# prannaykaul/lvc

Hardware: AMD Instinct MI355X
Metric: img/s COCO 800x1333 R50-FPN inference (GeneralizedRCNN.forward(batched_inputs) -> Instances, 1000 proposals, 100 detections) (higher is better)
Workload: dtype f32 (conv/GEMM inner products on the fp16 / bf16 matrix cores through fp32-accurate operand splits: two-way fp16 with main + cross fp32 accumulators for the 3x3 and wide 1x1 / FC layers, three-way bf16 for the rest; final boxes/scores closer to the fp64 evaluation than the reference's fp32 CPU path,; 1 GPU; COCO-detection R50-FPN inference, bs=8 synthetic 3x800x1333 per GPU, 1000 pre/post-NMS proposals per level/image, 80 classes, conditioned random-init weights; batch_per_gpu=8, global_batch=8, parallelism=dp1

## Files before the change

lvc_amd/_lib.py:

```python
import ctypes
import os

_HERE = os.path.dirname(os.path.abspath(__file__))
_SO = os.environ.get("LVC_AMD_LIB") or os.path.join(_HERE, "liblvc_amd.so")
_lib = None

c_void_p = ctypes.c_void_p
c_int = ctypes.c_int
c_float = ctypes.c_float
c_double = ctypes.c_double
c_longlong = ctypes.c_longlong


class LvcNativeError(RuntimeError):
    pass


def lib():
    global _lib
    if _lib is None:
        if not os.path.exists(_SO):
            raise ImportError(
                "lvc_amd: native library {} not found; build it with "
                "`python -c 'import __graft_entry__ as g; g.build()'` or `make -C lvc_amd/csrc` "
                "(there is no CPU fallback)".format(_SO)
            )
        L = ctypes.CDLL(_SO)
        L.lvc_last_error.restype = ctypes.c_char_p
        L.lvc_batched_nms_workspace_bytes.restype = c_longlong
        L.lvc_tta_merge_workspace_bytes.restype = c_longlong
        L.lvc_abi_version.restype = c_int
        L.lvc_set_wino_streamk.restype = None
        if os.environ.get("LVC_WINO_STREAMK", "0") != "0":
            L.lvc_set_wino_streamk(c_int(int(os.environ["LVC_WINO_STREAMK"])))
        L.lvc_set_nms_reduce_global.restype = None
        L.lvc_set_halo_test_hooks.restype = None
        if os.environ.get("LVC_NMS_REDUCE_GLOBAL", "0") != "0":
            L.lvc_set_nms_reduce_global(c_int(1))
        _lib = L
    return _lib


def check(status, what=""):
    if status != 0:
        msg = lib().lvc_last_error().decode("utf-8", "replace")
        lib().lvc_set_range_slot(0)
        raise LvcNativeError("{} failed (status {}): {}".format(what or "lvc_amd native call", status, msg))


def ptr(t):
    if t is None:
        return c_void_p(0)
    return c_void_p(t.data_ptr())


def current_stream(device=None):
    import torch

    return c_void_p(torch.cuda.current_stream(device).cuda_stream)
```

lvc_amd/csrc/boxes.hip:

```cpp
#include "common.h"
#include <stdlib.h>

typedef unsigned long long u64;

extern "C" int lvc_batched_nms(const float*, const float*, const int*, const int*, int, int, double, int,
                               int*, int*, void*, long long, void*);
extern "C" long long lvc_batched_nms_workspace_bytes(int, int);

#define MAXL 8

__device__ __forceinline__ unsigned int desc_key(float f) {
  if (f == 0.f) f = 0.f;
  unsigned int u = __float_as_uint(f);
  u ^= (u >> 31) ? 0xFFFFFFFFu : 0x80000000u;
  return ~u;
}

__device__ __forceinline__ int block_excl_scan_1024(int v, int* sh, int* total) {
  const int lane = threadIdx.x & 63, wave = threadIdx.x >> 6;
  int x = v;
#pragma unroll
  for (int o = 1; o < 64; o <<= 1) {
    int t = __shfl_up(x, o);
    if (lane >= o) x += t;
  }
  __syncthreads();
  if (lane == 63) sh[wave] = x;
  __syncthreads();
  if (threadIdx.x == 0) {
    int s = 0;
    for (int w = 0; w < 16; ++w) { int t = sh[w]; sh[w] = s; s += t; }
    sh[16] = s;
  }
  __syncthreads();
  *total = sh[16];
  return sh[wave] + x - v;
}

template <typename T>
__device__ __forceinline__ void bitonic_sort_lds(T* keys, int npad) {
  for (int k = 2; k <= npad; k <<= 1) {
    for (int j = k >> 1; j > 0; j >>= 1) {
      for (int t = threadIdx.x; t < npad / 2; t += blockDim.x) {
        int lo = ((t & ~(j - 1)) << 1) | (t & (j - 1));
        int hi = lo | j;
        bool up = (lo & k) == 0;
        T a = keys[lo], b = keys[hi];
        if ((a > b) == up) { keys[lo] = b; keys[hi] = a; }
      }
      __syncthreads();
    }
  }
}

struct RpnLevels {
  const float* logits[MAXL];
  const float* deltas[MAXL];
  int ld_logit[MAXL], ld_delta[MAXL];
  int H[MAXL], W[MAXL], stride[MAXL];
  int cand_off[MAXL + 1];
  long long key_off[MAXL + 1];
  const float* cell_anchors[MAXL];
  int L, A;
};

__device__ __forceinline__ void find_digit(const int* __restrict__ h, int krem, int* sh) {
  const int tid = threadIdx.x, lane = tid & 63, wave = tid >> 6;
  int x = 0, incl = 0;
  if (tid < 256) {
    x = h[tid];
    incl = x;
#pragma unroll
    for (int o = 1; o < 64; o <<= 1) {
      const int t = __shfl_up(incl, o);
      if (lane >= o) incl += t;
    }
    if (lane == 63) sh[wave] = incl;
  }
  __syncthreads();
  if (tid < 256) {
    int off = 0;
    for (int w = 0; w < wave; ++w) off += sh[w];
    incl += off;
    if (incl - x < krem && krem <= incl) { sh[8] = tid; sh[9] = incl - x; }
  }
  __syncthreads();
}

#define TOPK_PAD 2048
__global__ __launch_bounds__(1024) void rpn_topk_kernel(RpnLevels lv, int topk, unsigned int* __restrict__ wkeys,
                                                        float* __restrict__ cand_score,
                                                        int* __restrict__ cand_idx, int Ntot, int small_only) {
  __shared__ u64 sortbuf[TOPK_PAD];
  __shared__ int hist[256];
  __shared__ int sh[20];
  __shared__ int s_nlt;
  const int l = blockIdx.x, b = blockIdx.y, tid = threadIdx.x;
  const int A = lv.A, HW = lv.H[l] * lv.W[l], n = HW * A;
  if (n > small_only) return;
  const int k = topk < n ? topk : n;
  const int ld = lv.ld_logit[l];
  const float* lg = lv.logits[l] + (size_t)b * HW * ld;
  unsigned int* keys = wkeys + (size_t)b * lv.key_off[lv.L] + lv.key_off[l];
  const int npad = k <= 1024 ? 1024 : TOPK_PAD;

  if (tid < 256) hist[tid] = 0;
  __syncthreads();
  for (int i = tid; i < n; i += 1024) {
    int p = i / A, a = i - p * A;
    unsigned int key = desc_key(lg[(size_t)p * ld + a]);
    keys[i] = key;
    atomicAdd(&hist[key >> 24], 1);
  }
  __syncthreads();
  unsigned int prefix = 0, pmask = 0;
  int krem = k;
  for (int pass = 0; pass < 4; ++pass) {
    const int shift = 24 - 8 * pass;
    if (pass > 0) {
      if (tid < 256) hist[tid] = 0;
      __syncthreads();
      for (int i = tid; i < n; i += 1024) {
        unsigned int key = keys[i];
        if ((key & pmask) == prefix) atomicAdd(&hist[(key >> shift) & 255], 1);
      }
      __syncthreads();
    }
    find_digit(hist, krem, sh);
    prefix |= (unsigned int)sh[8] << shift;
    pmask |= 255u << shift;
    krem -= sh[9];
    __syncthreads();
  }
  const unsigned int T = prefix;
  const int need_eq = krem, n_lt = k - krem;
  for (int i = tid; i < npad; i += 1024) sortbuf[i] = ~0ull;
  if (tid == 0) s_nlt = 0;
  __syncthreads();
  int eq_base = 0;
  for (int i0 = 0; i0 < n; i0 += 1024) {
    const int i = i0 + tid;
    unsigned int key = i < n ? keys[i] : 0xFFFFFFFFu;
    bool is_lt = i < n && key < T;
    bool is_eq = i < n && key == T;
    if (is_lt) {
      int slot = atomicAdd(&s_nlt, 1);
      sortbuf[slot] = ((u64)key << 32) | (unsigned)i;
    }
    if (eq_base < need_eq) {
      int tot;
      int rank = eq_base + block_excl_scan_1024(is_eq ? 1 : 0, sh, &tot);
      if (is_eq && rank < need_eq) sortbuf[n_lt + rank] = ((u64)key << 32) | (unsigned)i;
      eq_base += tot;
    }
  }
  __syncthreads();
  bitonic_sort_lds(sortbuf, npad);
  for (int r = tid; r < k; r += 1024) {
    int i = (int)(sortbuf[r] & 0xFFFFFFFFu);
    int p = i / A, a = i - p * A;
    cand_idx[(size_t)b * Ntot + lv.cand_off[l] + r] = i;
    cand_score[(size_t)b * Ntot + lv.cand_off[l] + r] = lg[(size_t)p * ld + a];
  }
}

#define TK_SLICE 8192
#define TK_HSTRIDE 1040

__device__ __forceinline__ void topk_prefix(const int* __restrict__ H, int npass, int k, int* sh, unsigned int* prefix,
                                            int* krem) {
  unsigned int pf = 0;
  int kr = k;
  for (int ps = 0; ps < npass; ++ps) {
    find_digit(H + ps * 256, kr, sh);
    pf |= (unsigned int)sh[8] << (24 - 8 * ps);
    kr -= sh[9];
    __syncthreads();
  }
  *prefix = pf;
  *krem = kr;
}

__global__ __launch_bounds__(1024) void rpn_topk_phase_kernel(RpnLevels lv, int topk, unsigned int* __restrict__ wkeys,
                                                              int* __restrict__ hist_all, u64* __restrict__ ckeys,
                                                              int* __restrict__ ties, int Ntot, int phase) {
  __shared__ int hist[256];
  __shared__ int sh[16];
  const int slice = blockIdx.x, l = blockIdx.y, b = blockIdx.z, tid = threadIdx.x, lane = tid & 63;
  const int A = lv.A, HW = lv.H[l] * lv.W[l], n = HW * A;
  if (n <= TK_SLICE) return;
  const int i0 = slice * TK_SLICE;
  if (i0 >= n) return;
  const int i1 = min(n, i0 + TK_SLICE);
  const int k = topk < n ? topk : n;
  const int ld = lv.ld_logit[l];
  const float* lg = lv.logits[l] + (size_t)b * HW * ld;
  unsigned int* keys = wkeys + (size_t)b * lv.key_off[lv.L] + lv.key_off[l];
  int* H = hist_all + ((size_t)b * lv.L + l) * TK_HSTRIDE;
  unsigned int prefix;
  int krem;
  topk_prefix(H, phase < 4 ? phase : 4, k, sh, &prefix, &krem);
  if (phase < 4) {
    if (tid < 256) hist[tid] = 0;
    __syncthreads();
    const unsigned int pmask = phase ? 0xFFFFFFFFu << (32 - 8 * phase) : 0u;
    const int shift = 24 - 8 * phase;
    for (int ib = i0; ib < i1; ib += 1024) {
      const int i = ib + tid;
      unsigned int key = 0;
      bool act = false;
      if (i < i1) {
        if (phase == 0) {
          const int pp = i / A, a = i - pp * A;
          key = desc_key(lg[(size_t)pp * ld + a]);
          keys[i] = key;
        } else {
          key = keys[i];
        }
        act = (key & pmask) == prefix;
      }
      const unsigned int d = (key >> shift) & 255u;
      u64 m = __ballot(act);
      while (m) {
        const int first = __ffsll((long long)m) - 1;
        const unsigned int dd = (unsigned int)__shfl((int)d, first);
        const u64 same = __ballot(act && d == dd);
        if (lane == first) atomicAdd(&hist[dd], __popcll(same));
        m &= ~same;
      }
    }
    __syncthreads();
    if (tid < 256 && hist[tid]) atomicAdd(&H[phase * 256 + tid], hist[tid]);
  } else {
    const unsigned int T = prefix;
    u64* ck = ckeys + (size_t)b * Ntot + lv.cand_off[l];
    int* tl = ties + ((size_t)b * lv.L + l) * TOPK_PAD;
    for (int i = i0 + tid; i < i1; i += 1024) {
      const unsigned int key = keys[i];
      if (key < T) {
        const int slot = atomicAdd(&H[1024], 1);
        ck[slot] = ((u64)key << 32) | (unsigned)i;
      } else if (key == T) {
        const int slot = atomicAdd(&H[1025], 1);
        if (slot < TOPK_PAD) tl[slot] = i;
      }
    }
  }
}

__global__ __launch_bounds__(1024) void rpn_topk_final_kernel(RpnLevels lv, int topk, const unsigned int* __restrict__ wkeys,
                                                              const int* __restrict__ hist_all,
                                                              const u64* __restrict__ ckeys, const int* __restrict__ ties,
                                                              float* __restrict__ cand_score, int* __restrict__ cand_idx,
                                                              int Ntot) {
  __shared__ u64 sortbuf[TOPK_PAD];
  __shared__ unsigned int tiebuf[TOPK_PAD];
  __shared__ int sh[20];
  const int l = blockIdx.x, b = blockIdx.y, tid = threadIdx.x;
  const int A = lv.A, HW = lv.H[l] * lv.W[l], n = HW * A;
  if (n <= TK_SLICE) return;
  const int k = topk < n ? topk : n;
  const int ld = lv.ld_logit[l];
  const float* lg = lv.logits[l] + (size_t)b * HW * ld;
  const unsigned int* keys = wkeys + (size_t)b * lv.key_off[lv.L] + lv.key_off[l];
  const int* H = hist_all + ((size_t)b * lv.L + l) * TK_HSTRIDE;
  unsigned int T;
  int need_eq;
  topk_prefix(H, 4, k, sh, &T, &need_eq);
  const int n_lt = k - need_eq;
  const int npad = k <= 1024 ? 1024 : TOPK_PAD;
  const u64* ck = ckeys + (size_t)b * Ntot + lv.cand_off[l];
  for (int i = tid; i < npad; i += 1024) sortbuf[i] = i < n_lt ? ck[i] : ~0ull;
  const int tie_total = H[1025];
  __syncthreads();
  if (tie_total <= TOPK_PAD) {
    const int* tl = ties + ((size_t)b * lv.L + l) * TOPK_PAD;
    int tp = 64;
    while (tp < tie_total) tp <<= 1;
    for (int i = tid; i < tp; i += 1024) tiebuf[i] = i < tie_total ? (unsigned int)tl[i] : 0xFFFFFFFFu;
    __syncthreads();
    bitonic_sort_lds(tiebuf, tp);
    for (int r = tid; r < need_eq; r += 1024) sortbuf[n_lt + r] = ((u64)T << 32) | tiebuf[r];
  } else {
    int eq_base = 0;
    for (int i0 = 0; i0 < n && eq_base < need_eq; i0 += 1024) {
      const int i = i0 + tid;
      const bool is_eq = i < n && keys[i] == T;
      int tot;
      const int rank = eq_base + block_excl_scan_1024(is_eq ? 1 : 0, sh, &tot);
      if (is_eq && rank < need_eq) sortbuf[n_lt + rank] = ((u64)T << 32) | (unsigned)i;
      eq_base += tot;
    }
  }
  __syncthreads();
  bitonic_sort_lds(sortbuf, npad);
  for (int r = tid; r < k; r += 1024) {
    const int i = (int)(sortbuf[r] & 0xFFFFFFFFu);
    const int pp = i / A, a = i - pp * A;
    cand_idx[(size_t)b * Ntot + lv.cand_off[l] + r] = i;
    cand_score[(size_t)b * Ntot + lv.cand_off[l] + r] = lg[(size_t)pp * ld + a];
  }
}

__device__ __forceinline__ void apply_deltas(float bx1, float by1, float bx2, float by2, float d0, float d1,
                                             float d2, float d3, float wx, float wy, float ww, float wh,
                                             float scale_clamp, float* o) {
  const float widths = bx2 - bx1, heights = by2 - by1;
  const float ctr_x = bx1 + 0.5f * widths, ctr_y = by1 + 0.5f * heights;
  const float dx = d0 / wx, dy = d1 / wy;
  float dw = d2 / ww, dh = d3 / wh;
  dw = dw > scale_clamp ? scale_clamp : dw;
  dh = dh > scale_clamp ? scale_clamp : dh;
  const float pcx = dx * widths + ctr_x, pcy = dy * heights + ctr_y;
  const float pw = expf(dw) * widths, ph = expf(dh) * heights;
  o[0] = pcx - 0.5f * pw; o[1] = pcy - 0.5f * ph; o[2] = pcx + 0.5f * pw; o[3] = pcy + 0.5f * ph;
}
__device__ __forceinline__ float clampf(float v, float lo, float hi) {
  v = v < lo ? lo : v;
  return v > hi ? hi : v;
}


__global__ __launch_bounds__(1024) void rpn_decode_seg_kernel(RpnLevels lv, const float* __restrict__ cand_score,
                                                              const int* __restrict__ cand_idx, int Ntot,
                                                              const int* __restrict__ image_sizes, float scale_clamp,
                                                              float min_box_size, int SN, float* __restrict__ sboxes,
                                                              float* __restrict__ sscores, int* __restrict__ scount) {
  __shared__ int sh[20];
  const int l = blockIdx.x, b = blockIdx.y, tid = threadIdx.x;
  const int seg = b * lv.L + l;
  const float img_h = (float)image_sizes[b * 2 + 0], img_w = (float)image_sizes[b * 2 + 1];
  const int c_begin = lv.cand_off[l], c_end = lv.cand_off[l + 1];
  const int A = lv.A, W = lv.W[l], HW = lv.H[l] * W;
  int base = 0;
  for (int c0 = c_begin; c0 < c_end; c0 += 1024) {
    const int c = c0 + tid;
    bool ok = false;
    float box[4] = {0, 0, 0, 0};
    float score = 0.f;
    if (c < c_end) {
      const int i = cand_idx[(size_t)b * Ntot + c];
      score = cand_score[(size_t)b * Ntot + c];
      const int p = i / A, a = i - p * A;
      const int y = p / W, x = p - y * W;
      const float sx = (float)(x * lv.stride[l]), sy = (float)(y * lv.stride[l]);
      const float* ca = lv.cell_anchors[l] + a * 4;
      const float ax1 = sx + ca[0], ay1 = sy + ca[1], ax2 = sx + ca[2], ay2 = sy + ca[3];
      const float* d = lv.deltas[l] + ((size_t)b * HW + p) * lv.ld_delta[l] + a * 4;
      apply_deltas(ax1, ay1, ax2, ay2, d[0], d[1], d[2], d[3], 1.f, 1.f, 1.f, 1.f, scale_clamp, box);
      ok = isfinite(box[0]) && isfinite(box[1]) && isfinite(box[2]) && isfinite(box[3]) && isfinite(score);
      box[0] = clampf(box[0], 0.f, img_w); box[1] = clampf(box[1], 0.f, img_h);
      box[2] = clampf(box[2], 0.f, img_w); box[3] = clampf(box[3], 0.f, img_h);
      ok = ok && (box[2] - box[0] > min_box_size) && (box[3] - box[1] > min_box_size);
    }
    int tot;
    const int pos = base + block_excl_scan_1024(ok ? 1 : 0, sh, &tot);
    if (ok) {
      float* o = sboxes + ((size_t)seg * SN + pos) * 4;
      o[0] = box[0]; o[1] = box[1]; o[2] = box[2]; o[3] = box[3];
      sscores[(size_t)seg * SN + pos] = score;
    }
    base += tot;
  }
  if (tid == 0) scount[seg] = base;
}

#define MERGE_LDS_SCORES 8192
__global__ __launch_bounds__(1024) void rpn_merge_levels_kernel(const float* __restrict__ sboxes,
                                                                const float* __restrict__ sscores,
                                                                const int* __restrict__ keep,
                                                                const int* __restrict__ num_keep, int L, int SN,
                                                                int post_topk, float* __restrict__ pboxes,
                                                                float* __restrict__ plogits, int* __restrict__ out_count) {
  __shared__ int s_nk[MAXL + 1];
  __shared__ float s_sc[MERGE_LDS_SCORES];
  const int b = blockIdx.x, tid = threadIdx.x;
  if (tid == 0) {
    int acc = 0;
    for (int l = 0; l < L; ++l) { s_nk[l] = acc; acc += num_keep[b * L + l]; }
    s_nk[L] = acc;
  }
  __syncthreads();
  const int total = s_nk[L];
  const int nout = total < post_topk ? total : post_topk;
  const bool in_lds = total <= MERGE_LDS_SCORES;
  if (in_lds) {
    for (int e = tid; e < total; e += 1024) {
      int l = 0;
      while (e >= s_nk[l + 1]) ++l;
      const int seg = b * L + l;
      s_sc[e] = sscores[(size_t)seg * SN + keep[(size_t)seg * SN + (e - s_nk[l])]];
    }
    __syncthreads();
  }
  for (int e = tid; e < total; e += 1024) {
    int l = 0;
    while (e >= s_nk[l + 1]) ++l;
    const int t = e - s_nk[l];
    const int seg = b * L + l;
    const int j = keep[(size_t)seg * SN + t];
    const float s = sscores[(size_t)seg * SN + j];
    int rank = t;
    for (int m = 0; m < L; ++m) {
      if (m == l) continue;
      const int segm = b * L + m, n = s_nk[m + 1] - s_nk[m];
      int lo = 0, hi = n;
      while (lo < hi) {
        const int mid = (lo + hi) >> 1;
        const float sm = in_lds ? s_sc[s_nk[m] + mid] : sscores[(size_t)segm * SN + keep[(size_t)segm * SN + mid]];
        if (sm > s || (sm == s && m < l)) lo = mid + 1; else hi = mid;
      }
      rank += lo;
    }
    if (rank < post_topk) {
      *reinterpret_cast<float4*>(pboxes + ((size_t)b * post_topk + rank) * 4) =
          *reinterpret_cast<const float4*>(sboxes + ((size_t)seg * SN + j) * 4);
      plogits[(size_t)b * post_topk + rank] = s;
    }
  }
  for (int r = nout + tid; r < post_topk; r += 1024) {
    *reinterpret_cast<float4*>(pboxes + ((size_t)b * post_topk + r) * 4) = float4{0.f, 0.f, 0.f, 0.f};
    plogits[(size_t)b * post_topk + r] = 0.f;
  }
  if (tid == 0) out_count[b] = nout;
}


static long long align16(long long x) { return (x + 15) & ~15ll; }

struct RpnPlan {
  int Ntot;
  long long nkeys;
  long long off_keys, off_cscore, off_cidx, off_cboxes, off_cscores2, off_clevels, off_ccount, off_keep, off_hist, off_ckeys, off_ties, off_nms, total;
  long long off_sboxes, off_sscores, off_scount, off_skeep, off_snk, off_snms, snms_bytes;
  int max_slices, SN;
};
static RpnPlan rpn_plan(int B, int L, int A, const int* Hs, const int* Ws, int pre_topk) {
  RpnPlan p;
  p.Ntot = 0; p.nkeys = 0; p.max_slices = 0;
  for (int l = 0; l < L; ++l) {
    long long n = (long long)Hs[l] * Ws[l] * A;
    p.nkeys += n;
    p.Ntot += (int)(n < pre_topk ? n : pre_topk);
    if (n > TK_SLICE) { int sl = (int)((n + TK_SLICE - 1) / TK_SLICE); if (sl > p.max_slices) p.max_slices = sl; }
  }
  long long o = 0;
  p.off_keys = o; o = align16(o + (long long)B * p.nkeys * 4);
  p.off_cscore = o; o = align16(o + (long long)B * p.Ntot * 4);
  p.off_cidx = o; o = align16(o + (long long)B * p.Ntot * 4);
  p.off_cboxes = o; o = align16(o + (long long)B * p.Ntot * 16);
  p.off_cscores2 = o; o = align16(o + (long long)B * p.Ntot * 4);
  p.off_clevels = o; o = align16(o + (long long)B * p.Ntot * 4);
  p.off_ccount = o; o = align16(o + (long long)B * 4);
  p.off_keep = o; o = align16(o + (long long)B * p.Ntot * 4);
  p.off_hist = o; o = align16(o + (long long)B * L * TK_HSTRIDE * 4);
  p.off_ckeys = o; o = align16(o + (long long)B * p.Ntot * 8);
  p.off_ties = o; o = align16(o + (long long)B * L * TOPK_PAD * 4);
  p.off_nms = o; o = align16(o + lvc_batched_nms_workspace_bytes(B, p.Ntot));
  p.SN = 0;
  for (int l = 0; l < L; ++l) {
    long long n = (long long)Hs[l] * Ws[l] * A;
    const int c = (int)(n < pre_topk ? n : pre_topk);
    if (c > p.SN) p.SN = c;
  }
  const long long segs = (long long)B * L;
  p.off_sboxes = o; o = align16(o + segs * p.SN * 16);
  p.off_sscores = o; o = align16(o + segs * p.SN * 4);
  p.off_scount = o; o = align16(o + segs * 4);
  p.off_skeep = o; o = align16(o + segs * p.SN * 4);
  p.off_snk = o; o = align16(o + segs * 4);
  p.snms_bytes = lvc_batched_nms_workspace_bytes((int)segs, p.SN);
  p.off_snms = o; o = align16(o + p.snms_bytes);
  p.total = o;
  return p;
}

extern "C" long long lvc_rpn_proposals_workspace_bytes(int B, int L, int A, const int* Hs, const int* Ws,
                                                       int pre_nms_topk) {
  if (L < 1 || L > MAXL) return -1;
  return rpn_plan(B, L, A, Hs, Ws, pre_nms_topk).total;
}

extern "C" int lvc_rpn_proposals(const float* const* logits, const int* ld_logit, const float* const* deltas,
                                 const int* ld_delta, const float* const* cell_anchors, const int* Hs,
                                 const int* Ws, const int* strides, int L, int A, int B,
                                 const int* d_image_sizes, int pre_nms_topk, int post_nms_topk,
                                 double nms_thresh, float min_box_size, float scale_clamp,
                                 float* out_boxes, float* out_logits, int* d_out_count, void* workspace,
                                 long long workspace_bytes, void* stream) {
  LVC_CHECK_ARG(L >= 1 && L <= MAXL, "1..8 levels");
  LVC_CHECK_ARG(B > 0 && A > 0, "bad B/A");
  LVC_CHECK_ARG(pre_nms_topk > 0 && pre_nms_topk <= TOPK_PAD, "pre_nms_topk must be in 1..2048");
  LVC_CHECK_ARG(post_nms_topk > 0, "post_nms_topk must be positive");
  LVC_CHECK_ARG(logits && deltas && cell_anchors && Hs && Ws && strides && d_image_sizes && out_boxes &&
                    out_logits && d_out_count && workspace, "null pointer");
  RpnPlan p = rpn_plan(B, L, A, Hs, Ws, pre_nms_topk);
  LVC_CHECK_ARG(workspace_bytes >= p.total, "workspace too small");
  RpnLevels lv;
  memset(&lv, 0, sizeof lv);
  lv.L = L; lv.A = A;
  for (int l = 0; l < L; ++l) {
    lv.logits[l] = logits[l]; lv.deltas[l] = deltas[l];
    lv.ld_logit[l] = ld_logit[l]; lv.ld_delta[l] = ld_delta[l];
    lv.H[l] = Hs[l]; lv.W[l] = Ws[l]; lv.stride[l] = strides[l];
    lv.cell_anchors[l] = cell_anchors[l];
    long long n = (long long)Hs[l] * Ws[l] * A;
    lv.key_off[l + 1] = lv.key_off[l] + n;
    lv.cand_off[l + 1] = lv.cand_off[l] + (int)(n < pre_nms_topk ? n : pre_nms_topk);
  }
  char* ws = (char*)workspace;
  hipStream_t st = (hipStream_t)stream;
  unsigned int* keys = (unsigned int*)(ws + p.off_keys);
  float* cand_score = (float*)(ws + p.off_cscore);
  int* cand_idx = (int*)(ws + p.off_cidx);
  const bool multi = p.max_slices > 0;
  if (multi) {
    int* hist = (int*)(ws + p.off_hist);
    u64* ckeys = (u64*)(ws + p.off_ckeys);
    int* ties = (int*)(ws + p.off_ties);
    if (hipMemsetAsync(hist, 0, (size_t)B * L * TK_HSTRIDE * 4, st) != hipSuccess) {
      lvc_set_error("%s: hipMemsetAsync failed", __func__);
      return LVC_ERR_HIP;
    }
    for (int phase = 0; phase <= 4; ++phase)
      hipLaunchKernelGGL(rpn_topk_phase_kernel, dim3(p.max_slices, L, B), dim3(1024), 0, st, lv, pre_nms_topk, keys,
                         hist, ckeys, ties, p.Ntot, phase);
    hipLaunchKernelGGL(rpn_topk_final_kernel, dim3(L, B), dim3(1024), 0, st, lv, pre_nms_topk, keys, hist, ckeys, ties,
                       cand_score, cand_idx, p.Ntot);
  }
  hipLaunchKernelGGL(rpn_topk_kernel, dim3(L, B), dim3(1024), 0, st, lv, pre_nms_topk, keys, cand_score,
                     cand_idx, p.Ntot, multi ? TK_SLICE : 0x7FFFFFFF);
  LVC_CHECK_LAUNCH();
  float* sboxes = (float*)(ws + p.off_sboxes);
  float* sscores = (float*)(ws + p.off_sscores);
  int* scount = (int*)(ws + p.off_scount);
  int* skeep = (int*)(ws + p.off_skeep);
  int* snk = (int*)(ws + p.off_snk);
  hipLaunchKernelGGL(rpn_decode_seg_kernel, dim3(L, B), dim3(1024), 0, st, lv, cand_score, cand_idx, p.Ntot,
                     d_image_sizes, scale_clamp, min_box_size, p.SN, sboxes, sscores, scount);
  LVC_CHECK_LAUNCH();
  const int keep_per_level = post_nms_topk < p.SN ? post_nms_topk : p.SN;
  int rc = lvc_batched_nms(sboxes, sscores, nullptr, scount, B * L, p.SN, nms_thresh, keep_per_level, skeep, snk,
                           ws + p.off_snms, p.snms_bytes, stream);
  if (rc) return rc;
  hipLaunchKernelGGL(rpn_merge_levels_kernel, dim3(B), dim3(1024), 0, st, sboxes, sscores, skeep, snk, L, p.SN,
                     post_nms_topk, out_boxes, out_logits, d_out_count);
  LVC_CHECK_LAUNCH();
  return LVC_OK;
}

__global__ void assign_levels_kernel(const float* __restrict__ boxes, int R, int B, int min_level, int max_level,
                                     float canonical_box_size, float canonical_level, int* __restrict__ levels,
                                     float* __restrict__ rois) {
  const int i = blockIdx.x * blockDim.x + threadIdx.x;
  if (i >= R * B) return;
  const float4 bx = *reinterpret_cast<const float4*>(boxes + (size_t)i * 4);
  const float area = (bx.z - bx.x) * (bx.w - bx.y);
  const float size = sqrtf(area);
  float lvl = floorf(canonical_level + log2f(size / canonical_box_size + 1e-8f));
  lvl = lvl < (float)min_level ? (float)min_level : lvl;
  lvl = lvl > (float)max_level ? (float)max_level : lvl;
  levels[i] = (int)lvl - min_level;
  if (rois) {
    float* r = rois + (size_t)i * 5;
    r[0] = (float)(i / R); r[1] = bx.x; r[2] = bx.y; r[3] = bx.z; r[4] = bx.w;
  }
}

extern "C" int lvc_assign_levels_rois(const float* boxes, int B, int R, int min_level, int max_level,
                                      int canonical_box_size, int canonical_level, int* levels, float* rois,
                                      void* stream) {
  LVC_CHECK_ARG(B >= 0 && R >= 0, "negative size");
  if (B * R == 0) return LVC_OK;
  LVC_CHECK_ARG(boxes && levels, "null pointer");
  hipLaunchKernelGGL(assign_levels_kernel, dim3(lvc_cdiv(B * R, 256)), dim3(256), 0, (hipStream_t)stream, boxes, R,
                     B, min_level, max_level, (float)canonical_box_size, (float)canonical_level, levels, rois);
  LVC_CHECK_LAUNCH();
  return LVC_OK;
}

#define DET_TILE_ROWS 64
#define DET_MAX_COLS 97
__global__ __launch_bounds__(DET_TILE_ROWS) void det_row_stats_kernel(const float* __restrict__ cls_logits, int ld_cls, int K,
                                                                     int rows, float score_thresh, float* __restrict__ st_mx,
                                                                     float* __restrict__ st_inv, int* __restrict__ st_cnt,
                                                                     unsigned long long* __restrict__ st_mask) {
  __shared__ float tile[DET_TILE_ROWS * DET_MAX_COLS];
  const int r0 = blockIdx.x * DET_TILE_ROWS, tid = threadIdx.x;
  const int ncol = K + 1, pitch = ncol | 1;
  for (int i = tid; i < DET_TILE_ROWS * ncol; i += DET_TILE_ROWS) {
    const int rr = i / ncol, cc = i - rr * ncol;
    const int r = r0 + rr;
    tile[rr * pitch + cc] = r < rows ? cls_logits[(size_t)r * ld_cls + cc] : 0.f;
  }
  __syncthreads();
  const int r = r0 + tid;
  if (r >= rows) return;
  const float* lg = tile + tid * pitch;
  float mx = -INFINITY;
  for (int k = 0; k <= K; ++k) { float v = lg[k]; mx = v > mx ? v : mx; }
  float sum = 0.f;
  for (int k = 0; k <= K; ++k) sum += expf(lg[k] - mx);
  const float inv = 1.f / sum;
  int cnt = 0;
  unsigned long long m0 = 0, m1 = 0;
  for (int k = 0; k < K; ++k) {
    const bool hit = expf(lg[k] - mx) * inv > score_thresh;
    cnt += hit ? 1 : 0;
    if (hit) { if (k < 64) m0 |= 1ull << k; else m1 |= 1ull << (k - 64); }
  }
  st_mx[r] = mx; st_inv[r] = inv; st_cnt[r] = cnt;
  st_mask[2 * (size_t)r] = m0; st_mask[2 * (size_t)r + 1] = m1;
}

__global__ __launch_bounds__(1024) void det_candidates_kernel(
    const float* __restrict__ cls_logits, int ld_cls, const float* __restrict__ deltas, int ld_delta,
    int K, int cls_agnostic, const float* __restrict__ proposals, const int* __restrict__ prop_count, int R,
    const int* __restrict__ image_sizes, float wx, float wy, float ww, float wh, float scale_clamp,
    float score_thresh, int Nmax, float* __restrict__ cboxes, float* __restrict__ cscores,
    int* __restrict__ cclass, int* __restrict__ crow, int* __restrict__ ccount, int* __restrict__ status,
    const float* __restrict__ st_mx, const float* __restrict__ st_inv, const int* __restrict__ st_cnt,
    const unsigned long long* __restrict__ st_mask) {
  __shared__ int sh[20];
  const int b = blockIdx.x, tid = threadIdx.x;
  const int nrow = prop_count ? min(prop_count[b], R) : R;
  const float img_h = (float)image_sizes[b * 2 + 0], img_w = (float)image_sizes[b * 2 + 1];
  int base = 0;
  for (int r0 = 0; r0 < nrow; r0 += 1024) {
    const int r = r0 + tid;
    int cnt = 0;
    float mx = -INFINITY, inv = 0.f;
    const float* lg = cls_logits + ((size_t)b * R + (r < nrow ? r : 0)) * ld_cls;
    if (r < nrow && st_cnt) {
      const size_t gr = (size_t)b * R + r;
      mx = st_mx[gr]; inv = st_inv[gr]; cnt = st_cnt[gr];
    } else if (r < nrow) {
      for (int k = 0; k <= K; ++k) { float v = lg[k]; mx = v > mx ? v : mx; }
      float sum = 0.f;
      for (int k = 0; k <= K; ++k) sum += expf(lg[k] - mx);
      inv = 1.f / sum;
      for (int k = 0; k < K; ++k) cnt += (expf(lg[k] - mx) * inv > score_thresh) ? 1 : 0;
    }
    int tot;
    int pos = base + block_excl_scan_1024(cnt, sh, &tot);
    if (r < nrow && cnt > 0) {
      const float4 pb = *reinterpret_cast<const float4*>(proposals + ((size_t)b * R + r) * 4);
      const float* dl = deltas + ((size_t)b * R + r) * ld_delta;
      auto emit = [&](int k) {
        const float pr = expf(lg[k] - mx) * inv;
        if (pr > score_thresh) {
          if (pos < Nmax) {
            const float* d = dl + (cls_agnostic ? 0 : k * 4);
            float box[4];
            apply_deltas(pb.x, pb.y, pb.z, pb.w, d[0], d[1], d[2], d[3], wx, wy, ww, wh, scale_clamp, box);
            float* o = cboxes + ((size_t)b * Nmax + pos) * 4;
            o[0] = clampf(box[0], 0.f, img_w); o[1] = clampf(box[1], 0.f, img_h);
            o[2] = clampf(box[2], 0.f, img_w); o[3] = clampf(box[3], 0.f, img_h);
            cscores[(size_t)b * Nmax + pos] = pr;
            cclass[(size_t)b * Nmax + pos] = k;
            crow[(size_t)b * Nmax + pos] = r;
          }
          ++pos;
        }
      };
      if (st_mask) {
        for (int w = 0; w < 2; ++w) {
          unsigned long long m = st_mask[2 * ((size_t)b * R + r) + w];
          while (m) {
            emit(w * 64 + __ffsll((long long)m) - 1);
            m &= m - 1;
          }
        }
      } else {
        for (int k = 0; k < K; ++k) emit(k);
      }
    }
    base += tot;
  }
  if (tid == 0) {
    if (base > Nmax) { atomicOr(status, 2); base = Nmax; }
    ccount[b] = base;
  }
}

__global__ __launch_bounds__(256) void det_gather_kernel(
    const float* __restrict__ cboxes, const float* __restrict__ cscores, const int* __restrict__ cclass,
    const int* __restrict__ crow, const int* __restrict__ keep, const int* __restrict__ num_keep, int Nmax,
    int topk, const float* __restrict__ post, float* __restrict__ oboxes, float* __restrict__ oscores,
    int* __restrict__ oclasses, int* __restrict__ orows, int* __restrict__ ocount) {
  __shared__ int wsum[4];
  const int b = blockIdx.x, tid = threadIdx.x;
  const int nk = min(num_keep[b], topk);
  int base = 0;
  for (int r0 = 0; r0 < topk; r0 += 256) {
    const int r = r0 + tid;
    bool ok = false;
    float4 bx = {0, 0, 0, 0};
    float s = 0.f; int c = 0, row = 0;
    if (r < nk) {
      const int i = keep[(size_t)b * Nmax + r];
      bx = *reinterpret_cast<const float4*>(cboxes + ((size_t)b * Nmax + i) * 4);
      s = cscores[(size_t)b * Nmax + i]; c = cclass[(size_t)b * Nmax + i]; row = crow[(size_t)b * Nmax + i];
      ok = true;
      if (post) {
        const float sx = post[b * 4 + 0], sy = post[b * 4 + 1], oh = post[b * 4 + 2], ow = post[b * 4 + 3];
        bx.x = clampf(bx.x * sx, 0.f, ow); bx.y = clampf(bx.y * sy, 0.f, oh);
        bx.z = clampf(bx.z * sx, 0.f, ow); bx.w = clampf(bx.w * sy, 0.f, oh);
        ok = (bx.z - bx.x > 0.f) && (bx.w - bx.y > 0.f);
      }
    }
    const u64 bal = __ballot(ok);
    const int lane = tid & 63, wave = tid >> 6;
    __syncthreads();
    if (lane == 0) wsum[wave] = __popcll(bal);
    __syncthreads();
    int wbase = 0, tot = 0;
    for (int w = 0; w < 4; ++w) { if (w < wave) wbase += wsum[w]; tot += wsum[w]; }
    const int pos = base + wbase + __popcll(bal & ((1ull << lane) - 1ull));
    if (ok) {
      *reinterpret_cast<float4*>(oboxes + ((size_t)b * topk + pos) * 4) = bx;
      oscores[(size_t)b * topk + pos] = s; oclasses[(size_t)b * topk + pos] = c; orows[(size_t)b * topk + pos] = row;
    }
    base += tot;
  }
  __syncthreads();
  for (int r = base + tid; r < topk; r += 256) {
    float4 z = {0, 0, 0, 0};
    *reinterpret_cast<float4*>(oboxes + ((size_t)b * topk + r) * 4) = z;
    oscores[(size_t)b * topk + r] = 0.f; oclasses[(size_t)b * topk + r] = 0; orows[(size_t)b * topk + r] = 0;
  }
  if (tid == 0) ocount[b] = base;
}

struct DetPlan { long long off_cboxes, off_cscores, off_cclass, off_crow, off_ccount, off_keep, off_nk, off_nms, total; };
static DetPlan det_plan(int B, int Nmax) {
  DetPlan p; long long o = 0;
  p.off_cboxes = o; o = align16(o + (long long)B * Nmax * 16);
  p.off_cscores = o; o = align16(o + (long long)B * Nmax * 4);
  p.off_cclass = o; o = align16(o + (long long)B * Nmax * 4);
  p.off_crow = o; o = align16(o + (long long)B * Nmax * 4);
  p.off_ccount = o; o = align16(o + (long long)B * 4);
  p.off_keep = o; o = align16(o + (long long)B * Nmax * 4);
  p.off_nk = o; o = align16(o + (long long)B * 4);
  p.off_nms = o; o = align16(o + lvc_batched_nms_workspace_bytes(B, Nmax));
  p.total = o;
  return p;
}
extern "C" long long lvc_fast_rcnn_inference_workspace_bytes(int B, int max_candidates) {
  return det_plan(B, max_candidates).total;
}

extern "C" int lvc_fast_rcnn_inference(const float* cls_logits, int ld_cls, const float* deltas, int ld_delta,
                                       int K, int cls_agnostic, const float* proposals,
                                       const int* d_prop_count, int B, int R, const int* d_image_sizes,
                                       float wx, float wy, float ww, float wh, float scale_clamp,
                                       float score_thresh, double nms_thresh, int topk, int max_candidates,
                                       const float* d_post, float* out_boxes, float* out_scores,
                                       int* out_classes, int* out_rows, int* d_out_count, int* d_status,
                                       void* workspace, long long workspace_bytes, void* stream) {
  LVC_CHECK_ARG(B > 0 && R > 0 && K > 0 && topk > 0, "bad sizes");
  LVC_CHECK_ARG(max_candidates > 0, "max_candidates must be positive");
  LVC_CHECK_ARG(cls_logits && deltas && proposals && d_image_sizes && out_boxes && out_scores && out_classes &&
                    out_rows && d_out_count && d_status && workspace, "null pointer");
  DetPlan p = det_plan(B, max_candidates);
  LVC_CHECK_ARG(workspace_bytes >= p.total, "workspace too small");
  char* ws = (char*)workspace;
  hipStream_t st = (hipStream_t)stream;
  float* cboxes = (float*)(ws + p.off_cboxes);
  float* cscores = (float*)(ws + p.off_cscores);
  int* cclass = (int*)(ws + p.off_cclass);
  int* crow = (int*)(ws + p.off_crow);
  int* ccount = (int*)(ws + p.off_ccount);
  int* keep = (int*)(ws + p.off_keep);
  int* nk = (int*)(ws + p.off_nk);
  const long long rows = (long long)B * R;
  float* st_mx = nullptr; float* st_inv = nullptr; int* st_cnt = nullptr;
  unsigned long long* st_mask = nullptr;
  if (K + 1 < DET_MAX_COLS && rows * 28 + 64 <= p.total - p.off_nms) {
    st_mask = (unsigned long long*)(ws + p.off_nms);
    st_mx = (float*)(st_mask + 2 * rows);
    st_inv = st_mx + rows;
    st_cnt = (int*)(st_inv + rows);
    hipLaunchKernelGGL(det_row_stats_kernel, dim3((unsigned)lvc_cdiv64(rows, DET_TILE_ROWS)), dim3(DET_TILE_ROWS), 0, st,
                       cls_logits, ld_cls, K, (int)rows, score_thresh, st_mx, st_inv, st_cnt, st_mask);
    LVC_CHECK_LAUNCH();
  }
  hipLaunchKernelGGL(det_candidates_kernel, dim3(B), dim3(1024), 0, st, cls_logits, ld_cls, deltas, ld_delta, K,
                     cls_agnostic, proposals, d_prop_count, R, d_image_sizes, wx, wy, ww, wh, scale_clamp,
                     score_thresh, max_candidates, cboxes, cscores, cclass, crow, ccount, d_status, st_mx, st_inv, st_cnt, st_mask);
  LVC_CHECK_LAUNCH();
  int rc = lvc_batched_nms(cboxes, cscores, cclass, ccount, B, max_candidates, nms_thresh, topk, keep, nk,
                           ws + p.off_nms, p.total - p.off_nms, stream);
  if (rc) return rc;
  hipLaunchKernelGGL(det_gather_kernel, dim3(B), dim3(256), 0, st, cboxes, cscores, cclass, crow, keep, nk,
                     max_candidates, topk, d_post, out_boxes, out_scores, out_classes, out_rows, d_out_count);
  LVC_CHECK_LAUNCH();
  return LVC_OK;
}

__global__ void decode_boxes_kernel(const float* __restrict__ deltas, int ld, const float* __restrict__ boxes, int M,
                                    int R, const int* __restrict__ image_sizes, float wx, float wy, float ww, float wh,
                                    float scale_clamp, float* __restrict__ out) {
  const int i = blockIdx.x * blockDim.x + threadIdx.x;
  if (i >= M) return;
  const float4 b = *reinterpret_cast<const float4*>(boxes + (size_t)i * 4);
  const float* d = deltas + (size_t)i * ld;
  float o[4];
  apply_deltas(b.x, b.y, b.z, b.w, d[0], d[1], d[2], d[3], wx, wy, ww, wh, scale_clamp, o);
  if (image_sizes) {
    const int img = i / R;
    const float h = (float)image_sizes[img * 2], w = (float)image_sizes[img * 2 + 1];
    o[0] = clampf(o[0], 0.f, w); o[1] = clampf(o[1], 0.f, h); o[2] = clampf(o[2], 0.f, w); o[3] = clampf(o[3], 0.f, h);
  }
  float4 r = {o[0], o[1], o[2], o[3]};
  *reinterpret_cast<float4*>(out + (size_t)i * 4) = r;
}

extern "C" int lvc_decode_boxes(const float* deltas, int ld, const float* boxes, int M, int R, const int* d_image_sizes,
                                float wx, float wy, float ww, float wh, float scale_clamp, float* out, void* stream) {
  LVC_CHECK_ARG(M >= 0 && R > 0 && ld >= 4, "bad shape");
  if (M == 0) return LVC_OK;
  LVC_CHECK_ARG(deltas && boxes && out, "null pointer");
  hipLaunchKernelGGL(decode_boxes_kernel, dim3(lvc_cdiv(M, 256)), dim3(256), 0, (hipStream_t)stream, deltas, ld, boxes, M, R,
                     d_image_sizes, wx, wy, ww, wh, scale_clamp, out);
  LVC_CHECK_LAUNCH();
  return LVC_OK;
}
```

lvc_amd/csrc/nms.hip:

```cpp
#include "common.h"

typedef unsigned long long u64;

__device__ __forceinline__ unsigned int ordered_desc_key(float f) {
  if (f == 0.f) f = 0.f;
  unsigned int u = __float_as_uint(f);
  u ^= (u >> 31) ? 0xFFFFFFFFu : 0x80000000u;
  return ~u;
}

template <int NPAD>
__global__ __launch_bounds__(1024) void nms_prep_kernel(const float* __restrict__ boxes,
                                                        const float* __restrict__ scores,
                                                        const int* __restrict__ idxs,
                                                        const int* __restrict__ counts, int Nmax,
                                                        int* __restrict__ order,
                                                        float* __restrict__ sboxes,
                                                        int* __restrict__ sidx) {
  extern __shared__ __attribute__((aligned(16))) unsigned char dsm[];
  u64* keys = reinterpret_cast<u64*>(dsm);
  __shared__ float red[16];
  const int img = blockIdx.x;
  const int tid = threadIdx.x;
  int n = counts ? counts[img] : Nmax;
  if (n > Nmax) n = Nmax;
  const float* bx = boxes + (size_t)img * Nmax * 4;
  const float* sc = scores + (size_t)img * Nmax;
  const int* ix = idxs ? idxs + (size_t)img * Nmax : nullptr;

  float m = -INFINITY;
  for (int i = tid; i < n * 4; i += 1024) {
    float v = bx[i];
    m = v > m ? v : m;
  }
  for (int o = 32; o > 0; o >>= 1) {
    float t = __shfl_xor(m, o);
    m = t > m ? t : m;
  }
  if ((tid & 63) == 0) red[tid >> 6] = m;
  __syncthreads();
  if (tid < 64) {
    float v = tid < 16 ? red[tid] : -INFINITY;
    for (int o = 8; o > 0; o >>= 1) {
      float t = __shfl_xor(v, o);
      v = t > v ? t : v;
    }
    if (tid == 0) red[0] = v;
  }
  __syncthreads();
  const float maxp1 = red[0] + 1.0f;

  int npad = 1024;
  while (npad < n) npad <<= 1;
  if (npad > NPAD) npad = NPAD;
  for (int i = tid; i < npad; i += 1024)
    keys[i] = i < n ? (((u64)ordered_desc_key(sc[i]) << 32) | (unsigned)i) : ~0ull;
  __syncthreads();
  for (int k = 2; k <= npad; k <<= 1) {
    for (int j = k >> 1; j > 0; j >>= 1) {
      for (int t = tid; t < npad / 2; t += 1024) {
        int lo = ((t & ~(j - 1)) << 1) | (t & (j - 1));
        int hi = lo | j;
        bool up = (lo & k) == 0;
        u64 a = keys[lo], b = keys[hi];
        if ((a > b) == up) { keys[lo] = b; keys[hi] = a; }
      }
      __syncthreads();
    }
  }
  int* ord = order + (size_t)img * Nmax;
  float* sb = sboxes + (size_t)img * Nmax * 4;
  int* si = sidx + (size_t)img * Nmax;
  for (int r = tid; r < n; r += 1024) {
    int i = (int)(keys[r] & 0xFFFFFFFFu);
    ord[r] = i;
    int id = ix ? ix[i] : 0;
    float off = (float)id * maxp1;
    sb[r * 4 + 0] = bx[i * 4 + 0] + off;
    sb[r * 4 + 1] = bx[i * 4 + 1] + off;
    sb[r * 4 + 2] = bx[i * 4 + 2] + off;
    sb[r * 4 + 3] = bx[i * 4 + 3] + off;
    si[r] = id;
  }
}

#define NMS_MASK_STRIDE 96
#define NMS_TILE 16384
#define NMS_HEAD_MIN 2048
__global__ __launch_bounds__(64) void nms_mask_kernel(const float* __restrict__ sboxes,
                                                      const int* __restrict__ sidx,
                                                      const int* __restrict__ counts, int Nmax,
                                                      int nwords, double thr, u64* __restrict__ mask, int row0,
                                                      int rows_cap, const int* __restrict__ num_keep, int max_keep) {
  const int img = blockIdx.z;
  int n = counts ? counts[img] : Nmax;
  if (n > Nmax) n = Nmax;
  const int nend = n < row0 + rows_cap ? n : row0 + rows_cap;
  if (num_keep && num_keep[img] >= max_keep) return;
  const int nchunks = nend > row0 ? (nend - row0 + 63) >> 6 : 0;
  const int lane = threadIdx.x;
  const float* sb = sboxes + (size_t)img * Nmax * 4;
  const int* si = sidx + (size_t)img * Nmax;
  for (int ci = blockIdx.y; ci < nchunks; ci += gridDim.y) {
  const int i_me = row0 + ci * 64 + lane;
  float ix1 = 0, iy1 = 0, ix2 = 0, iy2 = 0; int iid = -1;
  if (i_me < nend) {
    const float4 b = *reinterpret_cast<const float4*>(sb + (size_t)i_me * 4);
    ix1 = b.x; iy1 = b.y; ix2 = b.z; iy2 = b.w; iid = si[i_me];
  }
  const float iarea_me = (ix2 - ix1) * (iy2 - iy1);
  const int rows = min(64, nend - (row0 + ci * 64));
  for (int wj = ci + blockIdx.x; wj < nchunks; wj += gridDim.x) {
    const int j_me = row0 + wj * 64 + lane;
    float jx1 = 0, jy1 = 0, jx2 = 0, jy2 = 0; int jid = -2;
    if (j_me < nend) {
      const float4 b = *reinterpret_cast<const float4*>(sb + (size_t)j_me * 4);
      jx1 = b.x; jy1 = b.y; jx2 = b.z; jy2 = b.w; jid = si[j_me];
    }
    const float jarea = (jx2 - jx1) * (jy2 - jy1);
    u64 my_word = 0;
    for (int r = 0; r < rows; ++r) {
      const float ax1 = __shfl(ix1, r), ay1 = __shfl(iy1, r), ax2 = __shfl(ix2, r), ay2 = __shfl(iy2, r);
      const float aarea = __shfl(iarea_me, r);
      const int aid = __shfl(iid, r);
      const float xx1 = ax1 < jx1 ? jx1 : ax1;
      const float yy1 = ay1 < jy1 ? jy1 : ay1;
      const float xx2 = jx2 < ax2 ? jx2 : ax2;
      const float yy2 = jy2 < ay2 ? jy2 : ay2;
      float w = xx2 - xx1; if (!(w > 0.f)) w = 0.f;
      float h = yy2 - yy1; if (!(h > 0.f)) h = 0.f;
      const float inter = w * h;
      const float ovr = inter / (aarea + jarea - inter);
      const bool hit = (j_me < nend) && (j_me != row0 + ci * 64 + r) && (aid == jid) && ((double)ovr > thr);
      const u64 word = __ballot(hit);
      if (lane == r) my_word = word;
    }
    if (i_me < nend) mask[((size_t)img * rows_cap + (i_me - row0)) * nwords + wj] = my_word;
  }
  }
}

__global__ __launch_bounds__(256) void nms_cross_kernel(const float* __restrict__ sboxes, const int* __restrict__ sidx,
                                                        const int* __restrict__ counts, int Nmax, int nwords, double thr,
                                                        const int* __restrict__ kept_pos, const int* __restrict__ num_keep,
                                                        int max_keep, int row0, int rows_cap, u64* __restrict__ removed_init) {
  const int w = blockIdx.x * 4 + (threadIdx.x >> 6), lane = threadIdx.x & 63, img = blockIdx.y;
  if (w >= nwords) return;
  int n = counts ? counts[img] : Nmax;
  if (n > Nmax) n = Nmax;
  const int nend = n < row0 + rows_cap ? n : row0 + rows_cap;
  const int nk = num_keep[img];
  u64* dst = removed_init + (size_t)img * nwords + w;
  if (row0 + w * 64 >= nend || nk >= max_keep) {
    if (lane == 0) *dst = 0ull;
    return;
  }
  const float* sb = sboxes + (size_t)img * Nmax * 4;
  const int* si = sidx + (size_t)img * Nmax;
  const int* kp = kept_pos + (size_t)img * Nmax;
  const int j_me = row0 + w * 64 + lane;
  float jx1 = 0, jy1 = 0, jx2 = 0, jy2 = 0; int jid = -2;
  if (j_me < nend) {
    const float4 b = *reinterpret_cast<const float4*>(sb + (size_t)j_me * 4);
    jx1 = b.x; jy1 = b.y; jx2 = b.z; jy2 = b.w; jid = si[j_me];
  }
  const float jarea = (jx2 - jx1) * (jy2 - jy1);
  bool dead = false;
  for (int i = 0; i < nk; ++i) {
    const int p = kp[i];
    const float4 a = *reinterpret_cast<const float4*>(sb + (size_t)p * 4);
    const int aid = si[p];
    const float aarea = (a.z - a.x) * (a.w - a.y);
    const float xx1 = a.x < jx1 ? jx1 : a.x;
    const float yy1 = a.y < jy1 ? jy1 : a.y;
    const float xx2 = jx2 < a.z ? jx2 : a.z;
    const float yy2 = jy2 < a.w ? jy2 : a.w;
    float ww = xx2 - xx1; if (!(ww > 0.f)) ww = 0.f;
    float hh = yy2 - yy1; if (!(hh > 0.f)) hh = 0.f;
    const float inter = ww * hh;
    const float ovr = inter / (aarea + jarea - inter);
    dead = dead || ((aid == jid) && ((double)ovr > thr));
  }
  const u64 word = __ballot(dead && j_me < nend);
  if (lane == 0) *dst = word;
}

#define NMS_MAX_WORDS 256
__global__ __launch_bounds__(64) void nms_reduce_kernel(const u64* __restrict__ mask,
                                                        const int* __restrict__ order,
                                                        const int* __restrict__ counts, int Nmax,
                                                        int nwords, int max_keep,
                                                        int* __restrict__ keep,
                                                        int* __restrict__ num_keep, int row0, int rows_cap,
                                                        const u64* __restrict__ removed_init, int* __restrict__ kept_pos,
                                                        int accumulate) {
  __shared__ u64 removed[NMS_MAX_WORDS];
  const int img = blockIdx.x, lane = threadIdx.x;
  int n = counts ? counts[img] : Nmax;
  if (n > Nmax) n = Nmax;
  const int nend = n < row0 + rows_cap ? n : row0 + rows_cap;
  int nk = accumulate ? num_keep[img] : 0;
  if (accumulate && (row0 >= nend || nk >= max_keep)) return;
  const u64* mk = mask + (size_t)img * rows_cap * nwords;
  const int* ord = order + (size_t)img * Nmax;
  int* kp = keep + (size_t)img * Nmax;
  int* kpos = kept_pos ? kept_pos + (size_t)img * Nmax : nullptr;
  for (int w = lane; w < nwords; w += 64) removed[w] = (removed_init && row0 > 0) ? removed_init[(size_t)img * nwords + w] : 0ull;
  __syncthreads();
  const int nchunks = nend > row0 ? (nend - row0 + 63) >> 6 : 0;
  for (int c = 0; c < nchunks && nk < max_keep; ++c) {
    const int row = row0 + c * 64 + lane;
    const u64 diag = row < nend ? mk[(size_t)(row - row0) * nwords + c] : 0ull;
    u64 alive = ~removed[c];
    const int valid = nend - (row0 + c * 64);
    if (valid < 64) alive &= ((1ull << valid) - 1ull);
    alive = ((u64)(unsigned)__builtin_amdgcn_readfirstlane((int)(unsigned)(alive >> 32)) << 32) |
            (unsigned)__builtin_amdgcn_readfirstlane((int)(unsigned)alive);
    const u64 col = diag & ((1ull << lane) - 1ull);
    u64 kept = 0;
    while (alive) {
      const bool und = (alive >> lane) & 1ull;
      const bool rem = und && (col & kept) != 0ull;
      const bool kp1 = und && !rem && (col & alive) == 0ull;
      const u64 bk = __ballot(kp1), br = __ballot(rem);
      kept |= bk;
      alive &= ~(bk | br);
    }
    if ((kept >> lane) & 1ull) {
      const int pos = nk + __popcll(kept & ((1ull << lane) - 1ull));
      if (pos < max_keep) {
        kp[pos] = ord[row];
        if (kpos) kpos[pos] = row;
      }
    }
    nk += __popcll(kept);
    for (int w0 = c + 1; w0 < nchunks; w0 += 64) {
      const int w = w0 + lane;
      const int wc = w < nwords ? w : nwords - 1;
      u64 acc = 0;
      u64 k = kept;
      while (k) {
        u64 v[24];
#pragma unroll
        for (int u = 0; u < 24; ++u) {
          const int i = k ? __ffsll((long long)k) - 1 : -1;
          k &= k - 1;
          const u64 x = mk[(size_t)(c * 64 + (i < 0 ? 0 : i)) * nwords + wc];
          v[u] = i < 0 ? 0ull : x;
        }
#pragma unroll
        for (int u = 0; u < 24; ++u) acc |= v[u];
      }
      if (w < nwords) removed[w] |= acc;
    }
    __syncthreads();
  }
  if (lane == 0) num_keep[img] = nk < max_keep ? nk : max_keep;
}

#define NMS_LDS_ROWS 1024
#define NMS_LDS_PITCH 17
__global__ __launch_bounds__(256) void nms_reduce_lds_kernel(const u64* __restrict__ mask, const int* __restrict__ order,
                                                             const int* __restrict__ counts, int Nmax, int nwords, int max_keep,
                                                             int* __restrict__ keep, int* __restrict__ num_keep, int rows_cap) {
  __shared__ u64 m[NMS_LDS_ROWS * NMS_LDS_PITCH];
  __shared__ int sord[NMS_LDS_ROWS];
  const int img = blockIdx.x, tid = threadIdx.x, lane = tid & 63;
  int n = counts ? counts[img] : Nmax;
  if (n > Nmax) n = Nmax;
  if (n > rows_cap) n = rows_cap;
  const u64* mk = mask + (size_t)img * rows_cap * nwords;
  const int* ord = order + (size_t)img * Nmax;
  const int nchunks = (n + 63) >> 6;
  for (int r = tid; r < n; r += 256) sord[r] = ord[r];
  const int total = n * nwords;
  for (int base = tid; base < total; base += 256 * 8) {
    u64 v[8];
#pragma unroll
    for (int j = 0; j < 8; ++j) {
      const int idx = base + j * 256;
      v[j] = idx < total ? mk[idx] : 0ull;
    }
#pragma unroll
    for (int j = 0; j < 8; ++j) {
      const int idx = base + j * 256;
      const int r = idx / nwords, w = idx - r * nwords;
      if (idx < total && w >= (r >> 6) && w < nchunks) m[r * NMS_LDS_PITCH + w] = v[j];
    }
  }
  __syncthreads();
  if (tid >= 64) return;
  int* kp = keep + (size_t)img * Nmax;
  u64 removed = 0;
  int nk = 0;
  const int w16 = lane & 15, g4 = lane >> 4;
  for (int c = 0; c < nchunks && nk < max_keep; ++c) {
    const int row = c * 64 + lane;
    const u64 diag = row < n ? m[row * NMS_LDS_PITCH + c] : 0ull;
    const u64 rem_c = ((u64)(unsigned)__builtin_amdgcn_readlane((int)(unsigned)(removed >> 32), c) << 32) |
                      (unsigned)__builtin_amdgcn_readlane((int)(unsigned)removed, c);
    u64 alive = ~rem_c;
    const int valid = n - c * 64;
    if (valid < 64) alive &= ((1ull << valid) - 1ull);
    const u64 col = diag & ((1ull << lane) - 1ull);
    u64 kept = 0;
    while (alive) {
      const bool und = (alive >> lane) & 1ull;
      const bool rem = und && (col & kept) != 0ull;
      const bool kp1 = und && !rem && (col & alive) == 0ull;
      const u64 bk = __ballot(kp1), br = __ballot(rem);
      kept |= bk;
      alive &= ~(bk | br);
    }
    if ((kept >> lane) & 1ull) {
      const int pos = nk + __popcll(kept & ((1ull << lane) - 1ull));
      if (pos < max_keep) kp[pos] = sord[row];
    }
    nk += __popcll(kept);
    if (c + 1 < nchunks) {
      u64 acc = 0;
#pragma unroll
      for (int i = 0; i < 64; i += 4) {
        const int r = i + g4;
        const u64 x = m[(c * 64 + r) * NMS_LDS_PITCH + w16];
        acc |= ((kept >> r) & 1ull) ? x : 0ull;
      }
      acc |= (u64)__shfl_xor((long long)acc, 16);
      acc |= (u64)__shfl_xor((long long)acc, 32);
      if (lane < 16 && lane > c) removed |= acc;
    }
  }
  if (lane == 0) num_keep[img] = nk < max_keep ? nk : max_keep;
}

__device__ __forceinline__ unsigned int ordered_asc_key(float f) {
  unsigned int u = __float_as_uint(f);
  return u ^ ((u >> 31) ? 0xFFFFFFFFu : 0x80000000u);
}
__device__ __forceinline__ float ordered_asc_value(unsigned int u) {
  u ^= (u >> 31) ? 0x80000000u : 0xFFFFFFFFu;
  return __uint_as_float(u);
}

__global__ __launch_bounds__(256) void nms_max_kernel(const float* __restrict__ boxes, const int* __restrict__ counts,
                                                      int Nmax, unsigned int* __restrict__ maxkey) {
  const int img = blockIdx.y;
  int n = counts ? counts[img] : Nmax;
  if (n > Nmax) n = Nmax;
  const float* bx = boxes + (size_t)img * Nmax * 4;
  float m = -INFINITY;
  for (int i = blockIdx.x * 256 + threadIdx.x; i < n * 4; i += gridDim.x * 256) {
    const float v = bx[i];
    m = v > m ? v : m;
  }
  for (int o = 32; o > 0; o >>= 1) {
    const float t = __shfl_xor(m, o);
    m = t > m ? t : m;
  }
  if ((threadIdx.x & 63) == 0) atomicMax(maxkey + img, ordered_asc_key(m));
}

__global__ __launch_bounds__(1024) void nms_sort_tile_kernel(const float* __restrict__ scores, const int* __restrict__ counts,
                                                             int Nmax, int npad, u64* __restrict__ keys, int mode, int klevel) {
  extern __shared__ __attribute__((aligned(16))) unsigned char dsm[];
  u64* tk = reinterpret_cast<u64*>(dsm);
  const int img = blockIdx.y, tile = blockIdx.x, tid = threadIdx.x;
  int n = counts ? counts[img] : Nmax;
  if (n > Nmax) n = Nmax;
  if (mode == 1 && n <= (klevel >> 1)) return;
  const int base = tile * NMS_TILE;
  u64* gk = keys + (size_t)img * npad + base;
  if (mode == 0) {
    const float* sc = scores + (size_t)img * Nmax;
    for (int i = tid; i < NMS_TILE; i += 1024) {
      const int gi = base + i;
      tk[i] = gi < n ? (((u64)ordered_desc_key(sc[gi]) << 32) | (unsigned)gi) : ~0ull;
    }
  } else {
    for (int i = tid; i < NMS_TILE; i += 1024) tk[i] = gk[i];
  }
  __syncthreads();
  const int k0 = mode == 0 ? 2 : klevel, k1 = mode == 0 ? NMS_TILE : klevel;
  for (int k = k0; k <= k1; k <<= 1) {
    for (int j = (k >> 1) < NMS_TILE ? (k >> 1) : (NMS_TILE >> 1); j > 0; j >>= 1) {
      for (int t = tid; t < NMS_TILE / 2; t += 1024) {
        const int lo = ((t & ~(j - 1)) << 1) | (t & (j - 1));
        const int hi = lo | j;
        const bool up = ((base + lo) & k) == 0;
        const u64 a = tk[lo], b = tk[hi];
        if ((a > b) == up) { tk[lo] = b; tk[hi] = a; }
      }
      __syncthreads();
    }
  }
  for (int i = tid; i < NMS_TILE; i += 1024) gk[i] = tk[i];
}

__global__ __launch_bounds__(256) void nms_sort_global_kernel(const int* __restrict__ counts, int Nmax, int npad,
                                                              u64* __restrict__ keys, int k, int j) {
  const int img = blockIdx.y;
  int n = counts ? counts[img] : Nmax;
  if (n > Nmax) n = Nmax;
  if (n <= (k >> 1)) return;
  u64* gk = keys + (size_t)img * npad;
  for (int t = blockIdx.x * 256 + threadIdx.x; t < npad / 2; t += gridDim.x * 256) {
    const int lo = ((t & ~(j - 1)) << 1) | (t & (j - 1));
    const int hi = lo | j;
    const bool up = (lo & k) == 0;
    const u64 a = gk[lo], b = gk[hi];
    if ((a > b) == up) { gk[lo] = b; gk[hi] = a; }
  }
}

__global__ __launch_bounds__(256) void nms_gather_kernel(const float* __restrict__ boxes, const int* __restrict__ idxs,
                                                         const int* __restrict__ counts, int Nmax, int npad,
                                                         const u64* __restrict__ keys, const unsigned int* __restrict__ maxkey,
                                                         int* __restrict__ order, float* __restrict__ sboxes,
                                                         int* __restrict__ sidx) {
  const int img = blockIdx.y;
  int n = counts ? counts[img] : Nmax;
  if (n > Nmax) n = Nmax;
  const float maxp1 = ordered_asc_value(maxkey[img]) + 1.0f;
  const float* bx = boxes + (size_t)img * Nmax * 4;
  const int* ix = idxs ? idxs + (size_t)img * Nmax : nullptr;
  const u64* gk = keys + (size_t)img * npad;
  int* ord = order + (size_t)img * Nmax;
  float* sb = sboxes + (size_t)img * Nmax * 4;
  int* si = sidx + (size_t)img * Nmax;
  for (int r = blockIdx.x * 256 + threadIdx.x; r < n; r += gridDim.x * 256) {
    const int i = (int)(gk[r] & 0xFFFFFFFFu);
    ord[r] = i;
    const int id = ix ? ix[i] : 0;
    const float off = (float)id * maxp1;
    sb[(size_t)r * 4 + 0] = bx[(size_t)i * 4 + 0] + off;
    sb[(size_t)r * 4 + 1] = bx[(size_t)i * 4 + 1] + off;
    sb[(size_t)r * 4 + 2] = bx[(size_t)i * 4 + 2] + off;
    sb[(size_t)r * 4 + 3] = bx[(size_t)i * 4 + 3] + off;
    si[r] = id;
  }
}

static int pad_pow2(int n) {
  int p = 1024;
  while (p < n) p <<= 1;
  return p;
}

static long long pad_pow2_ll(long long n) {
  long long p = NMS_TILE;
  while (p < n) p <<= 1;
  return p;
}

extern "C" long long lvc_batched_nms_workspace_bytes(int B, int Nmax) {
  const long long rows = Nmax < NMS_TILE ? Nmax : NMS_TILE;
  const long long nwords = (rows + 63) / 64;
  long long per = (long long)Nmax * 4 * 4  + (long long)Nmax * 4  +
                  (long long)Nmax * 4  + rows * nwords * 8 ;
  if (Nmax > NMS_TILE)
    per += (long long)Nmax * 4 + NMS_MAX_WORDS * 8 + pad_pow2_ll(Nmax) * 8 + 16;
  else if (Nmax > NMS_HEAD_MIN)
    per += (long long)Nmax * 4 + NMS_MAX_WORDS * 8 + 16;
  return (long long)B * per + 512;
}

static int g_nms_reduce_global = 0;
extern "C" void lvc_set_nms_reduce_global(int on) { g_nms_reduce_global = on; }

extern "C" int lvc_batched_nms(const float* boxes, const float* scores, const int* idxs,
                               const int* d_counts, int B, int Nmax, double iou_threshold,
                               int max_keep, int* keep, int* d_num_keep, void* workspace,
                               long long workspace_bytes, void* stream) {
  LVC_CHECK_ARG(B >= 0 && Nmax >= 0, "negative size");
  if (B == 0) return LVC_OK;
  LVC_CHECK_ARG(d_num_keep, "null d_num_keep");
  hipStream_t st = (hipStream_t)stream;
  if (Nmax == 0) {
    (void)hipMemsetAsync(d_num_keep, 0, sizeof(int) * B, st);
    return LVC_OK;
  }
  LVC_CHECK_ARG(boxes && scores && keep && workspace, "null pointer");
  LVC_CHECK_ARG(workspace_bytes >= lvc_batched_nms_workspace_bytes(B, Nmax), "workspace too small");
  LVC_CHECK_ARG(((uintptr_t)workspace & 15) == 0, "workspace must be 16-byte aligned");
  const int rows_cap = Nmax < NMS_TILE ? Nmax : NMS_TILE;
  const int nwords = (rows_cap + 63) / 64;
  char* ws = (char*)workspace;
  float* sboxes = (float*)ws; ws += (size_t)B * Nmax * 16;
  int* order = (int*)ws; ws += (size_t)B * Nmax * 4;
  int* sidx = (int*)ws; ws += (size_t)B * Nmax * 4;
  ws = (char*)(((uintptr_t)ws + 15) & ~(uintptr_t)15);
  u64* mask = (u64*)ws; ws += (size_t)B * rows_cap * nwords * 8;
  if (max_keep <= 0) max_keep = Nmax;
  const dim3 mask_grid(nwords < NMS_MASK_STRIDE ? nwords : NMS_MASK_STRIDE, nwords, B);

  if (Nmax <= NMS_TILE) {
    const int npad = pad_pow2(Nmax);
    const size_t lds = (size_t)npad * 8;
#define LAUNCH_PREP(NP)                                                                              \
  {                                                                                                  \
    (void)hipFuncSetAttribute((const void*)nms_prep_kernel<NP>, hipFuncAttributeMaxDynamicSharedMemorySize, \
                        (int)lds);                                                                   \
    hipLaunchKernelGGL(nms_prep_kernel<NP>, dim3(B), dim3(1024), lds, st, boxes, scores, idxs,       \
                       d_counts, Nmax, order, sboxes, sidx);                                         \
  }
    switch (npad) {
      case 1024: LAUNCH_PREP(1024); break;
      case 2048: LAUNCH_PREP(2048); break;
      case 4096: LAUNCH_PREP(4096); break;
      case 8192: LAUNCH_PREP(8192); break;
      default: LAUNCH_PREP(16384); break;
    }
#undef LAUNCH_PREP
    LVC_CHECK_LAUNCH();
    int head = ((8 * max_keep + 63) / 64) * 64;
    if (head < 1024) head = 1024;
    if (Nmax > NMS_HEAD_MIN && head * 2 <= Nmax) {
      int* kept_pos = (int*)ws; ws += (size_t)B * Nmax * 4;
      ws = (char*)(((uintptr_t)ws + 15) & ~(uintptr_t)15);
      u64* removed_init = (u64*)ws;
      if (hipMemsetAsync(d_num_keep, 0, sizeof(int) * B, st) != hipSuccess) {
        lvc_set_error("%s: hipMemsetAsync failed", __func__);
        return LVC_ERR_HIP;
      }
      const int hw = head / 64;
      hipLaunchKernelGGL(nms_mask_kernel, dim3(hw < NMS_MASK_STRIDE ? hw : NMS_MASK_STRIDE, hw, B), dim3(64), 0, st, sboxes, sidx,
                         d_counts, Nmax, hw, iou_threshold, mask, 0, head, (const int*)nullptr, max_keep);
      LVC_CHECK_LAUNCH();
      hipLaunchKernelGGL(nms_reduce_kernel, dim3(B), dim3(64), 0, st, mask, order, d_counts, Nmax, hw, max_keep, keep,
                         d_num_keep, 0, head, removed_init, kept_pos, 1);
      LVC_CHECK_LAUNCH();
      const int rest = Nmax - head, rw = (rest + 63) / 64;
      hipLaunchKernelGGL(nms_cross_kernel, dim3(lvc_cdiv(rw, 4), B), dim3(256), 0, st, sboxes, sidx, d_counts, Nmax, rw,
                         iou_threshold, kept_pos, d_num_keep, max_keep, head, rest, removed_init);
      LVC_CHECK_LAUNCH();
      hipLaunchKernelGGL(nms_mask_kernel, dim3(rw < NMS_MASK_STRIDE ? rw : NMS_MASK_STRIDE, rw < 16 ? rw : 16, B), dim3(64), 0, st, sboxes, sidx,
                         d_counts, Nmax, rw, iou_threshold, mask, head, rest, (const int*)d_num_keep, max_keep);
      LVC_CHECK_LAUNCH();
      hipLaunchKernelGGL(nms_reduce_kernel, dim3(B), dim3(64), 0, st, mask, order, d_counts, Nmax, rw, max_keep, keep,
                         d_num_keep, head, rest, removed_init, kept_pos, 1);
      LVC_CHECK_LAUNCH();
      return LVC_OK;
    }
    hipLaunchKernelGGL(nms_mask_kernel, mask_grid, dim3(64), 0, st, sboxes, sidx, d_counts, Nmax, nwords, iou_threshold,
                       mask, 0, rows_cap, (const int*)nullptr, max_keep);
    LVC_CHECK_LAUNCH();
    if (rows_cap <= NMS_LDS_ROWS && !g_nms_reduce_global)
      hipLaunchKernelGGL(nms_reduce_lds_kernel, dim3(B), dim3(256), 0, st, mask, order, d_counts, Nmax, nwords, max_keep, keep, d_num_keep,
                         rows_cap);
    else
      hipLaunchKernelGGL(nms_reduce_kernel, dim3(B), dim3(64), 0, st, mask, order, d_counts, Nmax, nwords, max_keep, keep,
                         d_num_keep, 0, rows_cap, (const u64*)nullptr, (int*)nullptr, 0);
    LVC_CHECK_LAUNCH();
    return LVC_OK;
  }

  int* kept_pos = (int*)ws; ws += (size_t)B * Nmax * 4;
  ws = (char*)(((uintptr_t)ws + 15) & ~(uintptr_t)15);
  u64* removed_init = (u64*)ws; ws += (size_t)B * NMS_MAX_WORDS * 8;
  const long long npad = pad_pow2_ll(Nmax);
  LVC_CHECK_ARG(npad <= (1ll << 30), "more than 2^30 boxes per image");
  u64* keys = (u64*)ws; ws += (size_t)B * npad * 8;
  unsigned int* maxkey = (unsigned int*)ws;
  if (hipMemsetAsync(maxkey, 0, sizeof(unsigned int) * B, st) != hipSuccess ||
      hipMemsetAsync(d_num_keep, 0, sizeof(int) * B, st) != hipSuccess) {
    lvc_set_error("%s: hipMemsetAsync failed", __func__);
    return LVC_ERR_HIP;
  }
  hipLaunchKernelGGL(nms_max_kernel, dim3(64, B), dim3(256), 0, st, boxes, d_counts, Nmax, maxkey);
  LVC_CHECK_LAUNCH();
  const size_t lds = (size_t)NMS_TILE * 8;
  (void)hipFuncSetAttribute((const void*)nms_sort_tile_kernel, hipFuncAttributeMaxDynamicSharedMemorySize, (int)lds);
  const int ntiles = (int)(npad / NMS_TILE);
  hipLaunchKernelGGL(nms_sort_tile_kernel, dim3(ntiles, B), dim3(1024), lds, st, scores, d_counts, Nmax, (int)npad, keys, 0, 0);
  LVC_CHECK_LAUNCH();
  for (long long k = 2ll * NMS_TILE; k <= npad; k <<= 1) {
    for (long long j = k >> 1; j >= NMS_TILE; j >>= 1) {
      hipLaunchKernelGGL(nms_sort_global_kernel, dim3(256, B), dim3(256), 0, st, d_counts, Nmax, (int)npad, keys, (int)k, (int)j);
      LVC_CHECK_LAUNCH();
    }
    hipLaunchKernelGGL(nms_sort_tile_kernel, dim3(ntiles, B), dim3(1024), lds, st, scores, d_counts, Nmax, (int)npad, keys, 1, (int)k);
    LVC_CHECK_LAUNCH();
  }
  hipLaunchKernelGGL(nms_gather_kernel, dim3(64, B), dim3(256), 0, st, boxes, idxs, d_counts, Nmax, (int)npad, keys, maxkey,
                     order, sboxes, sidx);
  LVC_CHECK_LAUNCH();
  for (int row0 = 0; row0 < Nmax; row0 += NMS_TILE) {
    if (row0 > 0) {
      hipLaunchKernelGGL(nms_cross_kernel, dim3(lvc_cdiv(nwords, 4), B), dim3(256), 0, st, sboxes, sidx, d_counts, Nmax,
                         nwords, iou_threshold, kept_pos, d_num_keep, max_keep, row0, rows_cap, removed_init);
      LVC_CHECK_LAUNCH();
    }
    hipLaunchKernelGGL(nms_mask_kernel, mask_grid, dim3(64), 0, st, sboxes, sidx, d_counts, Nmax, nwords, iou_threshold, mask,
                       row0, rows_cap, (const int*)d_num_keep, max_keep);
    LVC_CHECK_LAUNCH();
    hipLaunchKernelGGL(nms_reduce_kernel, dim3(B), dim3(64), 0, st, mask, order, d_counts, Nmax, nwords, max_keep, keep,
                       d_num_keep, row0, rows_cap, removed_init, kept_pos, 1);
    LVC_CHECK_LAUNCH();
  }
  return LVC_OK;
}
```

lvc_amd/kernels.py:

```python
import collections
import ctypes

import torch

from . import _lib
from ._lib import LvcNativeError, c_double, c_float, c_int, c_longlong, c_void_p, check, ptr

BK = 32
BN = 128


def _stream(t):
    return c_void_p(torch.cuda.current_stream(t.device).cuda_stream)


def _req_cuda(*ts):
    for t in ts:
        if t is not None and not t.is_cuda:
            raise RuntimeError("lvc_amd kernels need device tensors (got a CPU tensor); there is no CPU path")


class PackedConv:

    __slots__ = ("w", "scale", "shift", "K", "C", "R", "S", "stride", "pad", "Kg", "mode", "_w3", "_w2h", "_w2s", "two_acc",
# ... 783 lines not shown
    ok = (1 <= len(xs) <= 6 and _direct_f16_3x3(pc, C)
          and (pc.two_acc or pc.state["tier"] == 1 or HALO_S1 == 1)
          and pc.K in (128, 256) and pc.Kg == 9 * C
          and pred.mode == 0 and pred.R == 1 and pred.S == 1 and pred.stride == 1 and pred.pad == 0 and pred.C == pc.K and pred.Kg == pc.K
          and 1 <= pred.K <= 32 and pred.w.shape[0] >= 32 and pred.state["tier"] < 2
          and _level_maps_ok(xs, N, C, pc.K))
    if not ok:
        return None
    ms = [x.shape[0] * x.shape[1] * x.shape[2] for x in xs]
    if _outs is None:
        y = torch.zeros(sum(ms), pred.K, device=xs[0].device, dtype=torch.float32)
        outs, off = [], 0
        for x, m in zip(xs, ms):
            outs.append(y[off:off + m].view(x.shape[0], x.shape[1], x.shape[2], pred.K))
            off += m
    else:
        outs = _outs
    if CONV_WINO and WINO_RPN and HALO_S1 == 2 and pc.state["tier"] == 0:
        big, rest = _wino_levels(xs, pc.K)
        if big:
            u, scale = pack_wino(pc)
            pplanes = pred.split2h()
            pc.last_one = True
            pred.last_one = False
            for i in big:
                x, o = xs[i], outs[i]
                px = x.shape[0] * x.shape[1] * x.shape[2]
                _launch("f16x2_wino", 2.0 * px * pc.K * (C * 9 + pred.K), 4.0 * (px * C + px * pred.K + pc.K * (C * 9 + pred.K)), pc.slot,
                        "lvc_conv3x3_nhwc_wino_pred", lambda: _lib.lib().lvc_conv3x3_nhwc_wino_pred(
                            ptr(x), ptr(u), ptr(scale), ptr(pc.shift), ptr(o), c_int(N), c_int(x.shape[1]), c_int(x.shape[2]),
                            c_int(C), c_int(pc.K), c_int(u.shape[4]), c_int(1 if relu else 0), c_int(pred.K), ptr(pplanes),
                            ptr(pred.scale), ptr(pred.shift), c_int(pred.K), c_int(pred.w.shape[0]), c_int(pred.slot),
                            ptr(conv_workspace(x.device)), _stream(x)))
            if rest:
                sub = conv3x3_levels_pred([xs[i] for i in rest], pc, pred, relu=relu, _outs=[outs[i] for i in rest])
                assert sub is not None
            return outs
    L = len(xs)
    XP, IP = c_void_p * L, c_int * L
    xp, yp = XP(*[x.data_ptr() for x in xs]), XP(*[o.data_ptr() for o in outs])
    hs, ws = IP(*[x.shape[1] for x in xs]), IP(*[x.shape[2] for x in xs])
    pc.last_one = False
    pred.last_one = False
    planes, pplanes = pc.split2h(), pred.split2h()
    px = sum(ms)
    _launch("f16x2_halo", 2.0 * px * pc.K * (C * 9 + pred.K), 4.0 * (px * C + px * pred.K + pc.K * (C * 9 + pred.K)), pc.slot,
            "lvc_conv3x3_nhwc_f16_levels_pred", lambda: _lib.lib().lvc_conv3x3_nhwc_f16_levels_pred(
                c_int(0), xp, yp, hs, ws, c_int(L), ptr(planes), ptr(pc.scale), ptr(pc.shift), c_int(N),
                c_int(C), c_int(pc.K), c_int(pc.Kg), c_int(1 if relu else 0), ptr(pplanes),
                ptr(pred.scale), ptr(pred.shift), c_int(pred.K), c_int(pred.w.shape[0]),
                c_int(pred.K), c_int(pred.slot), ptr(conv_workspace(xs[0].device)), _stream(xs[0])))
    return outs


def pack_chain(pc_a, pc_b, state=None):
    assert pc_b.C == pc_a.K
    ch = PackedChain()
    ch.slot = _new_range_slot(ch)
    ch.state = state if state is not None else {"off": False}
    ch.wa, ch.sa = _chain_planes(pc_a)
    ch.wb, ch.sb = _chain_planes(pc_b)
    ch.ta, ch.tb = pc_a.shift, pc_b.shift
    ch.K1, ch.N1, ch.N2 = pc_a.C, pc_a.K, pc_b.K
    return ch


def conv1x1_chain(x, ch, residual=None, relu1=True, relu2=True, out1=None, out2=None):
    _req_cuda(x, residual)
    assert x.dtype == torch.float32 and x.is_contiguous() and x.shape[-1] >= ch.K1
    M = x.numel() // x.shape[-1]
    lead = tuple(x.shape[:-1])
    if out1 is None:
        out1 = torch.empty(lead + (ch.N1,), device=x.device, dtype=torch.float32)
    if out2 is None:
        out2 = torch.empty(lead + (ch.N2,), device=x.device, dtype=torch.float32)
    if residual is not None:
        assert residual.is_contiguous() and residual.dtype == torch.float32 and residual.numel() // residual.shape[-1] == M
    nbytes = 4.0 * (M * (ch.K1 + ch.N1 + ch.N2 + (ch.N1 if residual is not None else 0)) + ch.K1 * ch.N1 + ch.N1 * ch.N2)
    _launch("f16s1_chain", 2.0 * M * (ch.K1 * ch.N1 + ch.N1 * ch.N2), nbytes, ch.slot, "lvc_conv1x1_chain_nhwc_f16s1",
            lambda: _lib.lib().lvc_conv1x1_chain_nhwc_f16s1(
                ptr(x), c_int(x.shape[-1]), ptr(ch.wa), c_int(ch.wa.shape[1]), ptr(ch.sa), ptr(ch.ta), ptr(residual),
                c_int(residual.shape[-1] if residual is not None else 0), ptr(out1), c_int(out1.shape[-1]), c_int(1 if relu1 else 0),
                ptr(ch.wb), c_int(ch.wb.shape[1]), ptr(ch.sb), ptr(ch.tb), ptr(out2), c_int(out2.shape[-1]), c_int(1 if relu2 else 0),
                c_int(M), c_int(ch.K1), c_int(ch.N1), c_int(ch.N2), ptr(conv_workspace(x.device)), _stream(x)))
    return out1, out2


class PackedBneck:

    __slots__ = ("w", "s1", "t1", "s2", "t2", "s3", "t3", "cin", "proj", "slot", "state", "__weakref__")


BNECK = _os.environ.get("LVC_BNECK", "1") != "0"
BNECK_SHAPES = {(256, 64, 256, False), (64, 64, 256, True)}
_BNECK_IDX = {}


def _bneck_index(cin, proj, device):
    key = (cin, proj, str(device))
    if key in _BNECK_IDX:
        return _BNECK_IDX[key]
    import numpy as np

    lane = np.arange(64)
    rowl = (lane % 32)[:, None].repeat(8, 1)
    kpos = np.asarray(_PERM16)[(lane // 32)[:, None] * 8 + np.arange(8)[None]]

    def frags(specs):
        pl = np.stack([np.full((64, 8), s[0]) for s in specs])
        rows = np.stack([s[1] + rowl for s in specs])
        cols = np.stack([np.asarray(s[2])[kpos] for s in specs])
        return pl, rows, cols

    a16 = np.arange(16)
    p1 = [(pl, 32 * cb, 32 * c + 16 * sp + a16) for c in range(cin // 32) for sp in range(2) for cb in range(2) for pl in range(2)]

    def col2(ch, r, s_):
        return (ch // 32) * 288 + (r * 3 + s_) * 32 + ch % 32

    p2 = [(pl, 32 * cb, col2(16 * (u // 9) + a16, (u % 9) // 3, (u % 9) % 3)) for u in range(36) for cb in range(2) for pl in range(2)]
    p3 = [(pl, 32 * j, 64 * half + 16 * s + a16) for j in range(8) for half in range(2 if proj else 1) for s in range(4)
          for pl in range(2)]
    out = tuple(tuple(torch.from_numpy(np.ascontiguousarray(a)).to(device) for a in frags(sp)) for sp in (p1, p2, p3))
    _BNECK_IDX[key] = out
    return out


def pack_bottleneck(pc1, pc2, pc3, proj, state=None):
    assert pc1.R == 1 and pc2.R == 3 and pc2.S == 3 and pc2.pad == 1 and pc2.stride == 1 and pc3.R == 1 and pc1.stride == 1
    cin = pc1.C
    assert (cin, pc1.K, pc3.K, bool(proj)) in BNECK_SHAPES and pc2.C == 64 and pc2.K == 64 and pc3.C == (128 if proj else 64)
    dev = pc1.w.device
    bk = PackedBneck()
    bk.slot = _new_range_slot(bk)
    bk.state = state if state is not None else {"off": False}
    bk.cin, bk.proj = cin, bool(proj)
    parts = []
    affine = []
    for pc, (pl, rows, cols) in zip((pc1, pc2, pc3), _bneck_index(cin, bool(proj), dev)):
        nrows, Kg = pc.w.shape
        planes = torch.empty((2, nrows, Kg), device=dev, dtype=torch.float16)
        fac = torch.empty(nrows, device=dev, dtype=torch.float32)
        check(_lib.lib().lvc_split_weights_rowscaled(ptr(pc.w), c_int(nrows), c_int(Kg), ptr(planes), ptr(fac), _stream(pc.w)),
              "lvc_split_weights_rowscaled")
        parts.append(planes[pl, rows, cols].reshape(-1))
        fac = fac[: pc.K]
        affine.append(((fac * pc.scale) if pc.scale is not None else fac).contiguous())
        affine.append(pc.shift.contiguous() if pc.shift is not None else torch.zeros(pc.K, device=dev, dtype=torch.float32))
    bk.w = torch.cat(parts).contiguous()
    bk.s1, bk.t1, bk.s2, bk.t2, bk.s3, bk.t3 = affine
    return bk


def bottleneck_fused(x, bk, out=None):
    _req_cuda(x)
    assert x.dtype == torch.float32 and x.is_contiguous() and x.dim() == 4 and x.shape[-1] >= bk.cin
    N, H, W, ldx = x.shape
    if out is None:
        out = torch.empty(N, H, W, 256, device=x.device, dtype=torch.float32)
    M = N * H * W
    kk = bk.cin * 64 + 64 * 64 * 9 + 64 * 256 + (bk.cin * 256 if bk.proj else 0)
    _launch("f16s1_bneck", 2.0 * M * kk, 4.0 * (M * (bk.cin + 256) + kk), bk.slot, "lvc_bottleneck_nhwc_f16s1",
            lambda: _lib.lib().lvc_bottleneck_nhwc_f16s1(
                ptr(x), c_int(ldx), ptr(out), c_int(out.shape[-1]), c_int(N), c_int(H), c_int(W),
                c_int(bk.cin), c_int(1 if bk.proj else 0), ptr(bk.w), ptr(bk.s1), ptr(bk.t1), ptr(bk.s2),
                ptr(bk.t2), ptr(bk.s3), ptr(bk.t3), ptr(conv_workspace(x.device)), _stream(x)))
    return out


def split_planes_f16x2(w):
    _req_cuda(w)
    w = w.detach().float().contiguous()
    out = torch.empty((2,) + tuple(w.shape), device=w.device, dtype=torch.float16)
    check(_lib.lib().lvc_split_weights(ptr(w), c_longlong(w.numel()), c_int(2), ptr(out), ptr(_conv_error_view(w.device)), _stream(w)),
          "lvc_split_weights")
    return out


def stem_conv_pool(x4, pc, relu=True, second=None):
    _req_cuda(x4)
    assert x4.dim() == 4 and x4.shape[3] == 4 and x4.is_contiguous() and x4.dtype == torch.float32
    assert pc.mode == 1 and pc.K == 64 and pc.R == 7 and pc.stride == 2 and pc.pad == 3
    N, H, W, _ = x4.shape
    Ho, Wo = (H - 1) // 2 + 1, (W - 1) // 2 + 1
    Hp, Wp = (Ho - 1) // 2 + 1, (Wo - 1) // 2 + 1
    out = torch.empty(N, Hp, Wp, 64, device=x4.device, dtype=torch.float32)
    y2 = second(out.shape) if second is not None else None
    if y2 is not None:
        assert y2.shape == out.shape and y2.stride(3) == 1 and y2.stride(1) == Wp * y2.stride(2) and y2.stride(0) == Hp * y2.stride(1)
    if CONV_SPLIT == "f16x2":
        err = _conv_error_view(x4.device)
        st = _lib.lib().lvc_stem_conv_pool_nhwc4_f16x2(ptr(x4), ptr(pc.split2h()), ptr(pc.scale), ptr(pc.shift), ptr(out),
                                                       c_int(N), c_int(H), c_int(W), c_int(pc.w.shape[0]),
                                                       c_int(1 if relu else 0), ptr(err), ptr(y2),
                                                       c_int(y2.stride(2) if y2 is not None else 0), _stream(x4))
        check(st, "lvc_stem_conv_pool_nhwc4_f16x2")
        return out
    raise RuntimeError("the fused stem exists for the fp16 split only; BasicStem runs conv + max-pool as two launches otherwise")


def linear(x, pc, relu=False, split=None):
    M, Kin = x.shape
    y = conv2d_nhwc(x.view(M, 1, 1, Kin), pc, relu=relu, split=split)
    return y.view(M, pc.K)


def new_status(device):
    return torch.zeros(1, dtype=torch.int32, device=device)


def roi_align_forward(input, rois, spatial_scale, pooled_h, pooled_w, sampling_ratio, aligned, status=None):
    _req_cuda(input, rois)
    input = input.contiguous().float()
    rois = rois.contiguous().float()
    B, C, H, W = input.shape
    K = rois.shape[0]
    out = torch.empty(K, C, pooled_h, pooled_w, device=input.device, dtype=torch.float32)
    st = _lib.lib().lvc_roi_align_forward_nchw(
        ptr(input), ptr(rois), ptr(out), c_int(B), c_int(C), c_int(H), c_int(W), c_int(K),
        c_int(pooled_h), c_int(pooled_w), c_float(spatial_scale), c_int(sampling_ratio),
        c_int(1 if aligned else 0), ptr(status), _stream(input))
    check(st, "lvc_roi_align_forward_nchw")
    return out


ROI_ORDER_MIN = 1024


def roi_align_fpn_nhwc(feats, scales, rois, levels, pooled_h, pooled_w, sampling_ratio, aligned,
                       num_valid=None, status=None, order=None):
    _req_cuda(rois, *feats)
    L = len(feats)
    B, _, _, C = feats[0].shape
    K = rois.shape[0]
    rois = rois.contiguous().float()
    out = torch.empty(K, pooled_h, pooled_w, C, device=rois.device, dtype=torch.float32)
    FP = c_void_p * L
    IP = c_int * L
    FL = c_float * L
    fp = FP(*[f.data_ptr() for f in feats])
    hs = IP(*[f.shape[1] for f in feats])
    ws = IP(*[f.shape[2] for f in feats])
    sc = FL(*[float(s) for s in scales])
    for f in feats:
        assert f.is_contiguous() and f.dtype == torch.float32 and f.shape[0] == B and f.shape[3] == C
    if levels is not None:
        assert levels.dtype == torch.int32 and levels.is_contiguous()
    if order is not None:
        assert order.dtype == torch.int32 and order.is_contiguous() and order.numel() == K
    elif K >= ROI_ORDER_MIN:
        order = torch.empty(K, device=rois.device, dtype=torch.int32)
        if B <= 16:
            check(_lib.lib().lvc_roi_work_order_xcd(ptr(rois), ptr(levels), c_int(K), c_int(B), ptr(order), _stream(rois)), "lvc_roi_work_order_xcd")
        else:
            check(_lib.lib().lvc_roi_work_order(ptr(rois), ptr(levels), sc, c_int(L), c_int(K), c_int(pooled_h), ptr(order), _stream(rois)),
                  "lvc_roi_work_order")
    st = _lib.lib().lvc_roi_align_fpn_nhwc_ordered(
        fp, hs, ws, sc, c_int(L), c_int(B), c_int(C), ptr(rois), ptr(levels), ptr(num_valid), c_int(K),
        c_int(pooled_h), c_int(pooled_w), c_int(sampling_ratio), c_int(1 if aligned else 0), ptr(out),
        ptr(status), ptr(order), _stream(rois))
    check(st, "lvc_roi_align_fpn_nhwc")
    return out


def roi_align_backward(grad, rois, spatial_scale, pooled_h, pooled_w, batch_size, channels, height, width,
                       sampling_ratio, aligned, status=None):
    _req_cuda(grad, rois)
    grad = grad.contiguous().float()
    rois = rois.contiguous().float()
    K = rois.shape[0]
    assert grad.shape == (K, channels, pooled_h, pooled_w)
    gin = torch.empty(batch_size, channels, height, width, device=grad.device, dtype=torch.float32)
    st = _lib.lib().lvc_roi_align_backward_nchw(
        ptr(grad), ptr(rois), ptr(gin), c_int(batch_size), c_int(channels), c_int(height), c_int(width), c_int(K),
        c_int(pooled_h), c_int(pooled_w), c_float(spatial_scale), c_int(sampling_ratio),
        c_int(1 if aligned else 0), ptr(status), _stream(grad))
    check(st, "lvc_roi_align_backward_nchw")
    return gin


def roi_align_fpn_backward_nhwc(grad, shapes, scales, rois, levels, sampling_ratio, aligned, num_valid=None,
                                status=None):
    _req_cuda(grad, rois)
    grad = grad.contiguous().float()
    rois = rois.contiguous().float()
    K, ph, pw, C = grad.shape
    L = len(shapes)
    B = shapes[0][0]
    outs = [torch.empty(*sh, device=grad.device, dtype=torch.float32) for sh in shapes]
    FP = c_void_p * L
    IP = c_int * L
    FL = c_float * L
    if levels is not None:
        assert levels.dtype == torch.int32 and levels.is_contiguous()
    st = _lib.lib().lvc_roi_align_fpn_backward_nhwc(
        ptr(grad), FP(*[o.data_ptr() for o in outs]), IP(*[sh[1] for sh in shapes]), IP(*[sh[2] for sh in shapes]),
        FL(*[float(s) for s in scales]), c_int(L), c_int(B), c_int(C), ptr(rois), ptr(levels), ptr(num_valid),
        c_int(K), c_int(ph), c_int(pw), c_int(sampling_ratio), c_int(1 if aligned else 0), ptr(status),
        _stream(grad))
    check(st, "lvc_roi_align_fpn_backward_nhwc")
    return outs


def batched_nms_batch(boxes, scores, idxs, counts, iou_threshold, max_keep=0):
    _req_cuda(boxes, scores, idxs, counts)
    B, Nmax = scores.shape
    boxes = boxes.contiguous().float()
    scores = scores.contiguous().float()
    if idxs is not None:
        idxs = idxs.contiguous()
        assert idxs.dtype == torch.int32
    keep = torch.empty(B, Nmax, dtype=torch.int32, device=boxes.device)
    num_keep = torch.empty(B, dtype=torch.int32, device=boxes.device)
    wsb = _lib.lib().lvc_batched_nms_workspace_bytes(c_int(B), c_int(Nmax))
    ws = torch.empty(wsb, dtype=torch.uint8, device=boxes.device)
    st = _lib.lib().lvc_batched_nms(
        ptr(boxes), ptr(scores), ptr(idxs), ptr(counts), c_int(B), c_int(Nmax), c_double(iou_threshold),
        c_int(max_keep), ptr(keep), ptr(num_keep), ptr(ws), c_longlong(wsb), _stream(boxes))
    check(st, "lvc_batched_nms")
    return keep, num_keep


def batched_nms(boxes, scores, idxs, iou_threshold):
    n = boxes.shape[0]
    if n == 0:
        return torch.empty(0, dtype=torch.int64, device=boxes.device)
    idx32 = idxs.to(torch.int32)[None] if idxs is not None else None
    keep, nk = batched_nms_batch(boxes[None], scores[None], idx32, None, iou_threshold)
    return keep[0, : int(nk.item())].to(torch.int64)


def nms(boxes, scores, iou_threshold):
    return batched_nms(boxes, scores, None, iou_threshold)


SCALE_CLAMP = 4.135166556742356


def _arr(ctype, vals):
    return (ctype * len(vals))(*vals)


def rpn_proposals(logits, deltas, cell_anchors, strides, image_sizes, pre_nms_topk, post_nms_topk,
                  nms_thresh, min_box_size=0.0):
    L = len(logits)
    B, A = logits[0].shape[0], cell_anchors[0].shape[0]
    dev = logits[0].device
    _req_cuda(*logits, *deltas, *cell_anchors, image_sizes)
    for t in list(logits) + list(deltas):
        assert t.dtype == torch.float32 and t.stride(-1) == 1 and t.dim() == 4
        assert t.stride(2) == t.stride(3) * 0 + t.stride(2)
    Hs = [t.shape[1] for t in logits]
    Ws = [t.shape[2] for t in logits]
    for t, h, w in zip(list(logits) + list(deltas), Hs * 2, Ws * 2):
        assert t.stride(1) == w * t.stride(2) and t.stride(0) == h * w * t.stride(2), "need an NHWC channel slice"
    VP, IP = c_void_p * L, c_int * L
    lp = VP(*[t.data_ptr() for t in logits])
    dp = VP(*[t.data_ptr() for t in deltas])
    ap = VP(*[t.contiguous().data_ptr() for t in cell_anchors])
    ldl = IP(*[t.stride(2) for t in logits])
    ldd = IP(*[t.stride(2) for t in deltas])
    hs, ws_, st = IP(*Hs), IP(*Ws), IP(*strides)
    lib = _lib.lib()
    lib.lvc_rpn_proposals_workspace_bytes.restype = c_longlong
    nbytes = lib.lvc_rpn_proposals_workspace_bytes(c_int(B), c_int(L), c_int(A), hs, ws_, c_int(pre_nms_topk))
    ws = torch.empty(nbytes, dtype=torch.uint8, device=dev)
    boxes = torch.empty(B, post_nms_topk, 4, device=dev, dtype=torch.float32)
    olog = torch.empty(B, post_nms_topk, device=dev, dtype=torch.float32)
    count = torch.empty(B, dtype=torch.int32, device=dev)
    assert image_sizes.dtype == torch.int32 and image_sizes.is_contiguous()
    rc = lib.lvc_rpn_proposals(lp, ldl, dp, ldd, ap, hs, ws_, st, c_int(L), c_int(A), c_int(B), ptr(image_sizes),
                               c_int(pre_nms_topk), c_int(post_nms_topk), c_double(nms_thresh),
                               c_float(min_box_size), c_float(SCALE_CLAMP), ptr(boxes), ptr(olog), ptr(count),
                               ptr(ws), c_longlong(nbytes), _stream(boxes))
    check(rc, "lvc_rpn_proposals")
    return boxes, olog, count


def assign_levels_rois(boxes, min_level, max_level, canonical_box_size=224, canonical_level=4):
    _req_cuda(boxes)
    B, R, _ = boxes.shape
    boxes = boxes.contiguous()
    levels = torch.empty(B * R, dtype=torch.int32, device=boxes.device)
    rois = torch.empty(B * R, 5, dtype=torch.float32, device=boxes.device)
    rc = _lib.lib().lvc_assign_levels_rois(ptr(boxes), c_int(B), c_int(R), c_int(min_level), c_int(max_level),
                                           c_int(canonical_box_size), c_int(canonical_level), ptr(levels), ptr(rois),
                                           _stream(boxes))
    check(rc, "lvc_assign_levels_rois")
    return levels, rois


def fast_rcnn_inference(cls_logits, deltas, proposals, prop_count, image_sizes, num_classes, box_weights,
                        score_thresh, nms_thresh, topk, post=None, status=None, max_candidates=16384):
    _req_cuda(cls_logits, deltas, proposals, prop_count, image_sizes, post)
    B, R, _ = proposals.shape
    K = num_classes
    dev = proposals.device
    assert cls_logits.stride(1) == 1 and deltas.stride(1) == 1
    cls_agnostic = 1 if deltas.shape[1] == 4 else 0
    if status is None:
        status = new_status(dev)
    lib = _lib.lib()
    lib.lvc_fast_rcnn_inference_workspace_bytes.restype = c_longlong
    max_candidates = max(1, R * K) if max_candidates is None else min(max_candidates, max(1, R * K))
    nbytes = lib.lvc_fast_rcnn_inference_workspace_bytes(c_int(B), c_int(max_candidates))
    ws = torch.empty(nbytes, dtype=torch.uint8, device=dev)
    ob = torch.empty(B, topk, 4, device=dev, dtype=torch.float32)
    osc = torch.empty(B, topk, device=dev, dtype=torch.float32)
    ocl = torch.empty(B, topk, device=dev, dtype=torch.int32)
    orow = torch.empty(B, topk, device=dev, dtype=torch.int32)
    cnt = torch.empty(B, device=dev, dtype=torch.int32)
    wx, wy, ww, wh = box_weights
    rc = lib.lvc_fast_rcnn_inference(
        ptr(cls_logits), c_int(cls_logits.stride(0)), ptr(deltas), c_int(deltas.stride(0)), c_int(K),
        c_int(cls_agnostic), ptr(proposals.contiguous()), ptr(prop_count), c_int(B), c_int(R), ptr(image_sizes),
        c_float(wx), c_float(wy), c_float(ww), c_float(wh), c_float(SCALE_CLAMP), c_float(score_thresh),
        c_double(nms_thresh), c_int(topk), c_int(max_candidates), ptr(post), ptr(ob), ptr(osc), ptr(ocl), ptr(orow),
        ptr(cnt), ptr(status), ptr(ws), c_longlong(nbytes), _stream(proposals))
    check(rc, "lvc_fast_rcnn_inference")
    return ob, osc, ocl, orow, cnt


def preprocess_into(image, out_slot, mean, std):
    _req_cuda(image, out_slot)
    assert image.dim() == 3 and image.shape[0] == 3
    if image.dtype == torch.uint8:
        dt = 1
    else:
        image = image.float()
        dt = 0
    image = image.contiguous()
    Hp, Wp, four = out_slot.shape
    assert four == 4 and out_slot.is_contiguous()
    m = (c_float * 3)(*[float(v) for v in mean])
    s = (c_float * 3)(*[float(v) for v in std])
    rc = _lib.lib().lvc_preprocess_nhwc4(ptr(image), c_int(dt), c_int(image.shape[1]), c_int(image.shape[2]), m, s,
                                         ptr(out_slot), c_int(Hp), c_int(Wp), _stream(image))
    check(rc, "lvc_preprocess_nhwc4")


def preprocess_batch_into(images, out, mean, std):
    _req_cuda(out, *images)
    B = len(images)
    assert out.dim() == 4 and out.shape[0] == B and out.shape[3] == 4 and out.is_contiguous() and out.dtype == torch.float32
    u8 = images[0].dtype == torch.uint8
    imgs = []
    for im in images:
        assert im.dim() == 3 and im.shape[0] == 3
        if u8:
            assert im.dtype == torch.uint8
        else:
            im = im.float()
        imgs.append(im.contiguous())
    P = (c_void_p * B)(*[im.data_ptr() for im in imgs])
    hs = (c_int * B)(*[int(im.shape[1]) for im in imgs])
    ws = (c_int * B)(*[int(im.shape[2]) for im in imgs])
    m = (c_float * 3)(*[float(v) for v in mean])
    s_ = (c_float * 3)(*[float(v) for v in std])
    rc = _lib.lib().lvc_preprocess_batch_nhwc4(P, c_int(1 if u8 else 0), hs, ws, c_int(B), m, s_, ptr(out), c_int(out.shape[1]),
                                               c_int(out.shape[2]), _stream(out))
    check(rc, "lvc_preprocess_batch_nhwc4")
    return imgs


def resize_bilinear_u8(img, new_h, new_w, coeffs_fn, out_slot=None, mean=None, std=None):
    if not img.is_cuda:
        raise RuntimeError("resize_bilinear_u8 needs a device tensor (move the uint8 image first: 1 byte per sample)")
    img = img.contiguous()
    H, W, _ = img.shape
    dev = img.device
    xb = xk = yb = yk = tmp = None
    kxs = kys = 0
    if new_w != W:
        xb, xk, kxs = coeffs_fn(W, new_w, dev)
        tmp = torch.empty(H * new_w * 3, dtype=torch.uint8, device=dev)
    if new_h != H:
        yb, yk, kys = coeffs_fn(H, new_h, dev)
    out = torch.empty(new_h, new_w, 3, dtype=torch.uint8, device=dev)
    Hp = Wp = 0
    m = s = None
    if out_slot is not None:
        Hp, Wp, four = out_slot.shape
        assert four == 4 and out_slot.is_contiguous() and out_slot.dtype == torch.float32
        m = (c_float * 3)(*[float(v) for v in mean])
        s = (c_float * 3)(*[float(v) for v in std])
    rc = _lib.lib().lvc_resize_bilinear_u8(ptr(img), c_int(H), c_int(W), c_int(new_h), c_int(new_w), ptr(xb), ptr(xk),
                                           c_int(kxs), ptr(yb), ptr(yk), c_int(kys), ptr(tmp), ptr(out), ptr(out_slot),
                                           c_int(Hp), c_int(Wp), m, s, _stream(img))
    check(rc, "lvc_resize_bilinear_u8")
    return out


def tta_resize_u8(img, H, W, strides, hjobs, vjobs, mean, std):
    _req_cuda(img)
    assert img.dtype == torch.uint8
    hrows = []
    for xb, xk, ks, nw, tmp in hjobs:
        _req_cuda(xb, xk, tmp)
        assert tmp.numel() >= H * nw * 3
        hrows += [xb.data_ptr(), xk.data_ptr(), ks, nw, tmp.data_ptr()]
    vrows = []
    for hj, yb, yk, ks, nh, nw, u8, u8m, f, fm in vjobs:
        for o in (u8, u8m):
            assert o is None or (o.is_cuda and o.is_contiguous() and tuple(o.shape) == (nh, nw, 3) and o.dtype == torch.uint8)
        for o in (f, fm):
            assert o is None or (o.is_cuda and o.is_contiguous() and o.dim() == 3 and o.shape[2] == 4 and o.dtype == torch.float32)
        vrows += [hj, yb.data_ptr() if yb is not None else 0, yk.data_ptr() if yk is not None else 0, ks, nh, nw,
                  u8.data_ptr() if u8 is not None else 0, u8m.data_ptr() if u8m is not None else 0,
                  f.data_ptr() if f is not None else 0, f.shape[0] if f is not None else 0, f.shape[1] if f is not None else 0,
                  fm.data_ptr() if fm is not None else 0, fm.shape[0] if fm is not None else 0, fm.shape[1] if fm is not None else 0]
    hj = (c_longlong * max(1, len(hrows)))(*hrows)
    vj = (c_longlong * len(vrows))(*vrows)
    m = (c_float * 3)(*[float(v) for v in mean])
    s = (c_float * 3)(*[float(v) for v in std])
    sy, sx, sc = strides
    rc = _lib.lib().lvc_tta_resize_u8(ptr(img), c_int(H), c_int(W), c_longlong(sy), c_longlong(sx), c_longlong(sc), hj,
                                      c_int(len(hjobs)), vj, c_int(len(vjobs)), m, s, _stream(img))
    check(rc, "lvc_tta_resize_u8")


TRAIN_INPUT_LAUNCHES = []
TRAIN_INPUT_FIELDS = 24


class TrainInputWorkspace:

    def __init__(self, device):
        self.device = torch.device(device)
        self.host = self.dev = self.tmp = self.uploaded = None

    def wait_host(self):
        if self.uploaded is not None:
            self.uploaded.synchronize()

    def reserve(self, blob_bytes, tmp_bytes):
        if self.host is None or self.host.numel() < blob_bytes:
            n = max(blob_bytes * 3 // 2, 1 << 16)
            self.host = torch.empty(n, dtype=torch.uint8).pin_memory()
            self.dev = torch.empty(n, dtype=torch.uint8, device=self.device)
        if self.tmp is None or self.tmp.numel() < tmp_bytes:
            self.tmp = torch.empty(max(tmp_bytes * 3 // 2, 1 << 16), dtype=torch.uint8, device=self.device)


def train_input_u8(images, jobs, out, mean, std, coeffs_fn, want_u8=False, workspace=None):
    import numpy as np

    B = len(images)
    assert B == len(jobs) and B > 0
    _req_cuda(out, *images)
    assert out.dim() == 4 and out.shape[3] == 4 and out.is_contiguous() and out.dtype == torch.float32 and out.shape[0] >= B
    ws = workspace if workspace is not None else TrainInputWorkspace(out.device)
    tab = np.zeros((B, TRAIN_INPUT_FIELDS), np.int64)
    tables, off, tmp_off = [], B * TRAIN_INPUT_FIELDS * 8, 0
    u8 = []
    for i, (img, (x0, y0, cw, ch, nh, nw, flip)) in enumerate(zip(images, jobs)):
        assert img.dtype == torch.uint8 and img.dim() == 3 and img.shape[2] == 3 and img.device == out.device
        row = tab[i]
        row[0:6] = (img.data_ptr(), img.shape[0], img.shape[1], img.stride(0), img.stride(1), img.stride(2))
        row[6:12] = (x0, y0, cw, ch, nh, nw)
        row[12] = row[15] = -1
        for size_in, size_out, at in ((cw, nw, 12), (ch, nh, 15)):
            if size_in != size_out:
                b, k, ks = coeffs_fn(size_in, size_out)
                row[at], row[at + 1], row[at + 2] = off, off + b.nbytes, ks
                tables += [b, k]
                off += b.nbytes + k.nbytes
        row[18], row[19] = int(bool(flip)), i
        if want_u8:
            u8.append(torch.empty(nh, nw, 3, dtype=torch.uint8, device=out.device))
            row[20] = u8[-1].data_ptr()
        if nw != cw:
            row[21] = tmp_off
            tmp_off += (ch * nw * 3 + 255) & ~255
    ws.wait_host()
    ws.reserve(off, tmp_off)
    hb = ws.host.numpy()
    hb[:tab.nbytes] = tab.reshape(-1).view(np.uint8)
    at = tab.nbytes
    for t in tables:
        hb[at:at + t.nbytes] = np.ascontiguousarray(t, np.int32).reshape(-1).view(np.uint8)
        at += t.nbytes
    ws.dev[:off].copy_(ws.host[:off], non_blocking=True)
    ws.uploaded = torch.cuda.Event()
    ws.uploaded.record(torch.cuda.current_stream(out.device))
    m = (c_float * 3)(*[float(v) for v in mean])
    s = (c_float * 3)(*[float(v) for v in std])
    n = c_int(0)
    rc = _lib.lib().lvc_train_input_u8(ptr(ws.host), ptr(ws.dev), c_longlong(off), c_int(B), ptr(ws.tmp), c_longlong(ws.tmp.numel()),
                                       ptr(out), c_int(out.shape[0]), c_int(out.shape[1]), c_int(out.shape[2]), m, s, ctypes.byref(n),
                                       _stream(out))
    check(rc, "lvc_train_input_u8")
    TRAIN_INPUT_LAUNCHES.append(n.value)
    del TRAIN_INPUT_LAUNCHES[:-64]
    return u8 if want_u8 else None


TTA_PARAM_STRIDE = 16
TTA_MAX_STEPS = 4


def tta_merge(boxes, scores, classes, counts, params, tab, num_images, nmax, score_thresh, nms_thresh, topk):
    _req_cuda(boxes, scores, classes, counts, params, tab)
    A, T = scores.shape
    assert boxes.shape == (A, T, 4) and classes.shape == (A, T) and counts.shape == (A,) and params.shape == (A, TTA_PARAM_STRIDE)
    assert tab.shape == (num_images, 4) and tab.dtype == torch.int32 and params.dtype == torch.float32
    assert classes.dtype == torch.int32 and counts.dtype == torch.int32
    dev = boxes.device
    B = num_images
    ob = torch.empty(B, max(topk, 1), 4, device=dev, dtype=torch.float32)
    osc = torch.empty(B, max(topk, 1), device=dev, dtype=torch.float32)
    ocl = torch.empty(B, max(topk, 1), device=dev, dtype=torch.int32)
    cnt = torch.zeros(B, device=dev, dtype=torch.int32)
    if topk == 0 or B == 0:
        return ob[:, :0], osc[:, :0], ocl[:, :0], cnt
    wsb = _lib.lib().lvc_tta_merge_workspace_bytes(c_int(B), c_int(nmax))
    ws = torch.empty(wsb + 256, dtype=torch.uint8, device=dev)
    off = (-ws.data_ptr()) % 256
    ws = ws[off:off + wsb]
    rc = _lib.lib().lvc_tta_merge(ptr(boxes.contiguous()), ptr(scores.contiguous()), ptr(classes.contiguous()), ptr(counts), c_int(T),
                                  ptr(params), ptr(tab), c_int(B), c_int(nmax), c_float(score_thresh), c_double(nms_thresh),
                                  c_int(topk), ptr(ob), ptr(osc), ptr(ocl), ptr(cnt), ptr(ws), c_longlong(wsb), _stream(boxes))
    check(rc, "lvc_tta_merge")
    return ob, osc, ocl, cnt


def maxpool2d_nhwc(x, k, stride, pad):
    _req_cuda(x)
    assert x.is_contiguous() and x.dtype == torch.float32
    N, H, W, C = x.shape
    Ho = (H + 2 * pad - k) // stride + 1
    Wo = (W + 2 * pad - k) // stride + 1
    y = torch.empty(N, Ho, Wo, C, device=x.device, dtype=torch.float32)
    rc = _lib.lib().lvc_maxpool2d_nhwc(ptr(x), ptr(y), c_int(N), c_int(H), c_int(W), c_int(C), c_int(k), c_int(stride),
                                       c_int(pad), _stream(x))
    check(rc, "lvc_maxpool2d_nhwc")
    return y


def rownorm(x, mu=None, eps=1e-5, mode=0, out=None):
    _req_cuda(x, mu)
    assert x.dim() == 2 and x.stride(1) == 1 and x.dtype == torch.float32
    M, D = x.shape
    if out is None:
        out = torch.empty(M, D, device=x.device, dtype=torch.float32)
    rc = _lib.lib().lvc_rownorm(ptr(x), ptr(mu), ptr(out), c_int(M), c_int(D), c_int(x.stride(0)), c_int(out.stride(0)),
                                c_float(eps), c_int(mode), _stream(x))
    check(rc, "lvc_rownorm")
    return out


def rownorm_backward(x, dy, eps=1e-5, accumulate_into=None):
    _req_cuda(x, dy)
    x, dy = x.contiguous(), dy.contiguous()
    M, D = x.shape
    dx = accumulate_into if accumulate_into is not None else torch.empty_like(x)
    assert dx.is_contiguous() and dx.shape == x.shape
    check(_lib.lib().lvc_rownorm_backward(ptr(x), ptr(dy), ptr(dx), c_int(M), c_int(D), c_float(eps),
                                          c_int(1 if accumulate_into is not None else 0), _stream(x)), "lvc_rownorm_backward")
    return dx


def colmean(x):
    _req_cuda(x)
    assert x.dim() == 2 and x.stride(1) == 1 and x.dtype == torch.float32
    mu = torch.empty(x.shape[1], device=x.device, dtype=torch.float32)
    rc = _lib.lib().lvc_colmean(ptr(x), ptr(mu), c_int(x.shape[0]), c_int(x.shape[1]), c_int(x.stride(0)), _stream(x))
    check(rc, "lvc_colmean")
    return mu


def knn_topk_vote(sims, num_shots, shot_classes, det_classes, k):
    _req_cuda(sims, shot_classes, det_classes)
    Q = sims.shape[0]
    assert sims.stride(1) == 1 and shot_classes.dtype == torch.int64 and shot_classes.is_contiguous()
    top = torch.empty(Q, 10, dtype=torch.int64, device=sims.device)
    keep = torch.empty(Q, dtype=torch.int64, device=sims.device) if det_classes is not None else None
    if det_classes is not None:
        det_classes = det_classes.contiguous()
# ... 797 lines not shown
```

Before: 650.0 img/s.

## Replace radix top-k and NMS prep sort with histogram threshold selection

RPN per-level top-k now builds a 12-bit key histogram in parallel slices, then one workgroup per level finds the threshold bin and compacts only candidates at or below it into LDS before a bitonic sort. If a level's candidate count exceeds the LDS cap, it falls back to the old single-workgroup radix path. The head-form batched NMS likewise selects and sorts only the head candidates, and defers the full prep sort, gated on the head result. Detection row stats are split across more threads so the max and exp are computed once per element. The cost is extra kernels, workspace and flag plumbing, plus a slower path when the selected set overflows.

```diff
diff --git a/lvc_amd/_lib.py b/lvc_amd/_lib.py
--- a/lvc_amd/_lib.py
+++ b/lvc_amd/_lib.py
@@ -34,6 +34,9 @@
         if os.environ.get("LVC_WINO_STREAMK", "0") != "0":
             L.lvc_set_wino_streamk(c_int(int(os.environ["LVC_WINO_STREAMK"])))
         L.lvc_set_nms_reduce_global.restype = None
+        L.lvc_set_selection_fallback.restype = None
+        L.lvc_batched_nms_flag_offset.restype = c_longlong
+        L.lvc_rpn_proposals_flag_offset.restype = c_longlong
         L.lvc_set_halo_test_hooks.restype = None
         if os.environ.get("LVC_NMS_REDUCE_GLOBAL", "0") != "0":
             L.lvc_set_nms_reduce_global(c_int(1))
diff --git a/lvc_amd/csrc/boxes.hip b/lvc_amd/csrc/boxes.hip
--- a/lvc_amd/csrc/boxes.hip
+++ b/lvc_amd/csrc/boxes.hip
@@ -88,16 +88,12 @@
 }
 
 #define TOPK_PAD 2048
-__global__ __launch_bounds__(1024) void rpn_topk_kernel(RpnLevels lv, int topk, unsigned int* __restrict__ wkeys,
-                                                        float* __restrict__ cand_score,
-                                                        int* __restrict__ cand_idx, int Ntot, int small_only) {
-  __shared__ u64 sortbuf[TOPK_PAD];
-  __shared__ int hist[256];
-  __shared__ int sh[20];
-  __shared__ int s_nlt;
-  const int l = blockIdx.x, b = blockIdx.y, tid = threadIdx.x;
+__device__ __forceinline__ void topk_one_workgroup(const RpnLevels& lv, int l, int b, int topk, unsigned int* __restrict__ wkeys,
+                                                   float* __restrict__ cand_score, int* __restrict__ cand_idx, int Ntot,
+                                                   u64* sortbuf, int* hist, int* sh, int* s_nlt_p) {
+  int& s_nlt = *s_nlt_p;
+  const int tid = threadIdx.x;
   const int A = lv.A, HW = lv.H[l] * lv.W[l], n = HW * A;
-  if (n > small_only) return;
   const int k = topk < n ? topk : n;
   const int ld = lv.ld_logit[l];
   const float* lg = lv.logits[l] + (size_t)b * HW * ld;
@@ -162,6 +158,18 @@
     cand_idx[(size_t)b * Ntot + lv.cand_off[l] + r] = i;
     cand_score[(size_t)b * Ntot + lv.cand_off[l] + r] = lg[(size_t)p * ld + a];
   }
+}
+
+__global__ __launch_bounds__(1024) void rpn_topk_kernel(RpnLevels lv, int topk, unsigned int* __restrict__ wkeys,
+                                                        float* __restrict__ cand_score,
+                                                        int* __restrict__ cand_idx, int Ntot, int small_only) {
+  __shared__ u64 sortbuf[TOPK_PAD];
+  __shared__ int hist[256];
+  __shared__ int sh[20];
+  __shared__ int s_nlt;
+  const int l = blockIdx.x, b = blockIdx.y;
+  if (lv.H[l] * lv.W[l] * lv.A > small_only) return;
+  topk_one_workgroup(lv, l, b, topk, wkeys, cand_score, cand_idx, Ntot, sortbuf, hist, sh, &s_nlt);
 }
 
 #define TK_SLICE 8192
@@ -302,6 +310,121 @@
   }
 }
 
+#define SEL_SLICE 16384
+#define SEL_BITS 12
+#define SEL_BINS (1 << SEL_BITS)
+#define SEL_CAP 4096
+
+__global__ __launch_bounds__(1024) void rpn_keyhist_kernel(RpnLevels lv, unsigned int* __restrict__ wkeys,
+                                                           int* __restrict__ slabs, int max_slices) {
+  __shared__ int hist[SEL_BINS];
+  const int slice = blockIdx.x, l = blockIdx.y, b = blockIdx.z, tid = threadIdx.x;
+  const int A = lv.A, HW = lv.H[l] * lv.W[l], n = HW * A;
+  const int i0 = slice * SEL_SLICE;
+  if (i0 >= n) return;
+  const int i1 = min(n, i0 + SEL_SLICE);
+  const int ld = lv.ld_logit[l];
+  const float* lg = lv.logits[l] + (size_t)b * HW * ld;
+  unsigned int* keys = wkeys + (size_t)b * lv.key_off[lv.L] + lv.key_off[l];
+  for (int i = tid; i < SEL_BINS; i += 1024) hist[i] = 0;
+  __syncthreads();
+  for (int i = i0 + tid; i < i1; i += 1024) {
+    const int pp = i / A, a = i - pp * A;
+    const unsigned int key = desc_key(lg[(size_t)pp * ld + a]);
+    keys[i] = key;
+    atomicAdd(&hist[key >> (32 - SEL_BITS)], 1);
+  }
+  __syncthreads();
+  int* slab = slabs + (((size_t)b * lv.L + l) * max_slices + slice) * SEL_BINS;
+  for (int i = tid; i < SEL_BINS; i += 1024) slab[i] = hist[i];
+}
+
+__device__ __forceinline__ void find_threshold_bin(const int h[4], int k, int* sh) {
+  const int mine = h[0] + h[1] + h[2] + h[3];
+  int tot;
+  const int ex = block_excl_scan_1024(mine, sh, &tot);
+  if (ex < k && k <= ex + mine) {
+    int c = ex, bin = -1, incl = 0;
+#pragma unroll
+    for (int j = 0; j < 4; ++j) {
+      if (bin < 0) {
+        if (c + h[j] >= k) { bin = j; incl = c + h[j]; } else c += h[j];
+      }
+    }
+    sh[17] = threadIdx.x * 4 + bin;
+    sh[18] = incl;
+  }
+  __syncthreads();
+}
+
+__global__ __launch_bounds__(1024) void rpn_select_kernel(RpnLevels lv, int topk, unsigned int* __restrict__ wkeys,
+                                                          const int* __restrict__ slabs, int max_slices,
+                                                          float* __restrict__ cand_score, int* __restrict__ cand_idx,
+                                                          int Ntot, int* __restrict__ flags) {
+  __shared__ u64 sortbuf[SEL_CAP];
+  __shared__ int hist[256];
+  __shared__ int sh[20];
+  __shared__ int s_cnt;
+  const int l = blockIdx.x, b = blockIdx.y, tid = threadIdx.x, lane = tid & 63;
+  const int A = lv.A, HW = lv.H[l] * lv.W[l], n = HW * A;
+  const int seg = b * lv.L + l;
+  if (n <= 0) { if (tid == 0) flags[seg] = 0; return; }
+  const int k = topk < n ? topk : n;
+  const int nsl = (n + SEL_SLICE - 1) / SEL_SLICE;
+  const int* slab = slabs + ((size_t)seg * max_slices) * SEL_BINS;
+  int h[4] = {0, 0, 0, 0};
+  for (int s = 0; s < nsl; ++s) {
+    const int4 v = *reinterpret_cast<const int4*>(slab + (size_t)s * SEL_BINS + tid * 4);
+    h[0] += v.x; h[1] += v.y; h[2] += v.z; h[3] += v.w;
+  }
+  if (tid == 0) s_cnt = 0;
+  find_threshold_bin(h, k, sh);
+  const unsigned int tbin = (unsigned int)sh[17];
+  const int m = sh[18];
+  if (m > SEL_CAP) {
+    if (tid == 0) flags[seg] = 1;
+    __syncthreads();
+    topk_one_workgroup(lv, l, b, topk, wkeys, cand_score, cand_idx, Ntot, sortbuf, hist, sh, &s_cnt);
+    return;
+  }
+  if (tid == 0) flags[seg] = 0;
+  const unsigned int* keys = wkeys + (size_t)b * lv.key_off[lv.L] + lv.key_off[l];
+  int npad = 1024;
+  while (npad < m) npad <<= 1;
+  for (int i = m + tid; i < npad; i += 1024) sortbuf[i] = ~0ull;
+  for (int i0 = 0; i0 < n; i0 += 4096) {
+    unsigned int key[4];
+#pragma unroll
+    for (int u = 0; u < 4; ++u) {
+      const int i = i0 + u * 1024 + tid;
+      key[u] = i < n ? keys[i] : 0xFFFFFFFFu;
+    }
+#pragma unroll
+    for (int u = 0; u < 4; ++u) {
+      const int i = i0 + u * 1024 + tid;
+      const bool hit = i < n && (key[u] >> (32 - SEL_BITS)) <= tbin;
+      const u64 bal = __ballot(hit);
+      if (bal) {
+        int base = 0;
+        if (lane == 0) base = atomicAdd(&s_cnt, __popcll(bal));
+        base = __shfl(base, 0);
+        const int slot = base + __popcll(bal & ((1ull << lane) - 1ull));
+        if (hit && slot < SEL_CAP) sortbuf[slot] = ((u64)key[u] << 32) | (unsigned)i;
+      }
+    }
+  }
+  __syncthreads();
+  bitonic_sort_lds(sortbuf, npad);
+  const int ld = lv.ld_logit[l];
+  const float* lg = lv.logits[l] + (size_t)b * HW * ld;
+  for (int r = tid; r < k; r += 1024) {
+    const int i = (int)(sortbuf[r] & 0xFFFFFFFFu);
+    const int pp = i / A, a = i - pp * A;
+    cand_idx[(size_t)b * Ntot + lv.cand_off[l] + r] = i;
+    cand_score[(size_t)b * Ntot + lv.cand_off[l] + r] = lg[(size_t)pp * ld + a];
+  }
+}
+
 __device__ __forceinline__ void apply_deltas(float bx1, float by1, float bx2, float by2, float d0, float d1,
                                              float d2, float d3, float wx, float wy, float ww, float wh,
                                              float scale_clamp, float* o) {
@@ -433,13 +556,16 @@
   long long nkeys;
   long long off_keys, off_cscore, off_cidx, off_cboxes, off_cscores2, off_clevels, off_ccount, off_keep, off_hist, off_ckeys, off_ties, off_nms, total;
   long long off_sboxes, off_sscores, off_scount, off_skeep, off_snk, off_snms, snms_bytes;
-  int max_slices, SN;
+  long long off_slabs, off_flags;
+  int max_slices, sel_slices, SN;
 };
 static RpnPlan rpn_plan(int B, int L, int A, const int* Hs, const int* Ws, int pre_topk) {
   RpnPlan p;
-  p.Ntot = 0; p.nkeys = 0; p.max_slices = 0;
+  p.Ntot = 0; p.nkeys = 0; p.max_slices = 0; p.sel_slices = 1;
   for (int l = 0; l < L; ++l) {
     long long n = (long long)Hs[l] * Ws[l] * A;
+    const int ssl = (int)((n + SEL_SLICE - 1) / SEL_SLICE);
+    if (ssl > p.sel_slices) p.sel_slices = ssl;
     p.nkeys += n;
     p.Ntot += (int)(n < pre_topk ? n : pre_topk);
     if (n > TK_SLICE) { int sl = (int)((n + TK_SLICE - 1) / TK_SLICE); if (sl > p.max_slices) p.max_slices = sl; }
@@ -471,6 +597,8 @@
   p.off_snk = o; o = align16(o + segs * 4);
   p.snms_bytes = lvc_batched_nms_workspace_bytes((int)segs, p.SN);
   p.off_snms = o; o = align16(o + p.snms_bytes);
+  p.off_slabs = o; o = align16(o + segs * p.sel_slices * SEL_BINS * 4);
+  p.off_flags = o; o = align16(o + segs * 4);
   p.total = o;
   return p;
 }
@@ -480,6 +608,13 @@
   if (L < 1 || L > MAXL) return -1;
   return rpn_plan(B, L, A, Hs, Ws, pre_nms_topk).total;
 }
+
+extern "C" long long lvc_rpn_proposals_flag_offset(int B, int L, int A, const int* Hs, const int* Ws, int pre_nms_topk) {
+  if (L < 1 || L > MAXL) return -1;
+  return rpn_plan(B, L, A, Hs, Ws, pre_nms_topk).off_flags;
+}
+
+extern "C" int lvc_get_selection_fallback(void);
 
 extern "C" int lvc_rpn_proposals(const float* const* logits, const int* ld_logit, const float* const* deltas,
                                  const int* ld_delta, const float* const* cell_anchors, const int* Hs,
@@ -514,6 +649,12 @@
   float* cand_score = (float*)(ws + p.off_cscore);
   int* cand_idx = (int*)(ws + p.off_cidx);
   const bool multi = p.max_slices > 0;
+  if (!lvc_get_selection_fallback()) {
+    int* slabs = (int*)(ws + p.off_slabs);
+    hipLaunchKernelGGL(rpn_keyhist_kernel, dim3(p.sel_slices, L, B), dim3(1024), 0, st, lv, keys, slabs, p.sel_slices);
+    hipLaunchKernelGGL(rpn_select_kernel, dim3(L, B), dim3(1024), 0, st, lv, pre_nms_topk, keys, slabs, p.sel_slices,
+                       cand_score, cand_idx, p.Ntot, (int*)(ws + p.off_flags));
+  } else {
   if (multi) {
     int* hist = (int*)(ws + p.off_hist);
     u64* ckeys = (u64*)(ws + p.off_ckeys);
@@ -530,6 +671,7 @@
   }
   hipLaunchKernelGGL(rpn_topk_kernel, dim3(L, B), dim3(1024), 0, st, lv, pre_nms_topk, keys, cand_score,
                      cand_idx, p.Ntot, multi ? TK_SLICE : 0x7FFFFFFF);
+  }
   LVC_CHECK_LAUNCH();
   float* sboxes = (float*)(ws + p.off_sboxes);
   float* sscores = (float*)(ws + p.off_sscores);
@@ -579,37 +721,49 @@
   return LVC_OK;
 }
 
-#define DET_TILE_ROWS 64
+#define DET_TILE_ROWS 32
+#define DET_STATS_THREADS 256
 #define DET_MAX_COLS 97
-__global__ __launch_bounds__(DET_TILE_ROWS) void det_row_stats_kernel(const float* __restrict__ cls_logits, int ld_cls, int K,
-                                                                     int rows, float score_thresh, float* __restrict__ st_mx,
-                                                                     float* __restrict__ st_inv, int* __restrict__ st_cnt,
-                                                                     unsigned long long* __restrict__ st_mask) {
+__global__ __launch_bounds__(DET_STATS_THREADS) void det_row_stats_kernel(const float* __restrict__ cls_logits, int ld_cls, int K,
+                                                                         int rows, float score_thresh, float* __restrict__ st_mx,
+                                                                         float* __restrict__ st_inv, int* __restrict__ st_cnt,
+                                                                         unsigned long long* __restrict__ st_mask) {
   __shared__ float tile[DET_TILE_ROWS * DET_MAX_COLS];
+  __shared__ float s_mx[DET_TILE_ROWS];
   const int r0 = blockIdx.x * DET_TILE_ROWS, tid = threadIdx.x;
   const int ncol = K + 1, pitch = ncol | 1;
-  for (int i = tid; i < DET_TILE_ROWS * ncol; i += DET_TILE_ROWS) {
+  for (int i = tid; i < DET_TILE_ROWS * ncol; i += DET_STATS_THREADS) {
     const int rr = i / ncol, cc = i - rr * ncol;
     const int r = r0 + rr;
     tile[rr * pitch + cc] = r < rows ? cls_logits[(size_t)r * ld_cls + cc] : 0.f;
   }
   __syncthreads();
+  if (tid < DET_TILE_ROWS) {
+    const float* lg = tile + tid * pitch;
+    float mx = -INFINITY;
+    for (int k = 0; k <= K; ++k) { float v = lg[k]; mx = v > mx ? v : mx; }
+    s_mx[tid] = mx;
+  }
+  __syncthreads();
+  for (int i = tid; i < DET_TILE_ROWS * ncol; i += DET_STATS_THREADS) {
+    const int rr = i / ncol, cc = i - rr * ncol;
+    tile[rr * pitch + cc] = expf(tile[rr * pitch + cc] - s_mx[rr]);
+  }
+  __syncthreads();
   const int r = r0 + tid;
-  if (r >= rows) return;
-  const float* lg = tile + tid * pitch;
-  float mx = -INFINITY;
-  for (int k = 0; k <= K; ++k) { float v = lg[k]; mx = v > mx ? v : mx; }
+  if (tid >= DET_TILE_ROWS || r >= rows) return;
+  const float* ex = tile + tid * pitch;
   float sum = 0.f;
-  for (int k = 0; k <= K; ++k) sum += expf(lg[k] - mx);
+  for (int k = 0; k <= K; ++k) sum += ex[k];
   const float inv = 1.f / sum;
   int cnt = 0;
   unsigned long long m0 = 0, m1 = 0;
   for (int k = 0; k < K; ++k) {
-    const bool hit = expf(lg[k] - mx) * inv > score_thresh;
+    const bool hit = ex[k] * inv > score_thresh;
     cnt += hit ? 1 : 0;
     if (hit) { if (k < 64) m0 |= 1ull << k; else m1 |= 1ull << (k - 64); }
   }
-  st_mx[r] = mx; st_inv[r] = inv; st_cnt[r] = cnt;
+  st_mx[r] = s_mx[tid]; st_inv[r] = inv; st_cnt[r] = cnt;
   st_mask[2 * (size_t)r] = m0; st_mask[2 * (size_t)r + 1] = m1;
 }
 
@@ -776,12 +930,12 @@
   const long long rows = (long long)B * R;
   float* st_mx = nullptr; float* st_inv = nullptr; int* st_cnt = nullptr;
   unsigned long long* st_mask = nullptr;
-  if (K + 1 < DET_MAX_COLS && rows * 28 + 64 <= p.total - p.off_nms) {
+  if (!lvc_get_selection_fallback() && K + 1 < DET_MAX_COLS && rows * 28 + 64 <= p.total - p.off_nms) {
     st_mask = (unsigned long long*)(ws + p.off_nms);
     st_mx = (float*)(st_mask + 2 * rows);
     st_inv = st_mx + rows;
     st_cnt = (int*)(st_inv + rows);
-    hipLaunchKernelGGL(det_row_stats_kernel, dim3((unsigned)lvc_cdiv64(rows, DET_TILE_ROWS)), dim3(DET_TILE_ROWS), 0, st,
+    hipLaunchKernelGGL(det_row_stats_kernel, dim3((unsigned)lvc_cdiv64(rows, DET_TILE_ROWS)), dim3(DET_STATS_THREADS), 0, st,
                        cls_logits, ld_cls, K, (int)rows, score_thresh, st_mx, st_inv, st_cnt, st_mask);
     LVC_CHECK_LAUNCH();
   }
diff --git a/lvc_amd/csrc/nms.hip b/lvc_amd/csrc/nms.hip
--- a/lvc_amd/csrc/nms.hip
+++ b/lvc_amd/csrc/nms.hip
@@ -9,25 +9,10 @@
   return ~u;
 }
 
-template <int NPAD>
-__global__ __launch_bounds__(1024) void nms_prep_kernel(const float* __restrict__ boxes,
-                                                        const float* __restrict__ scores,
-                                                        const int* __restrict__ idxs,
-                                                        const int* __restrict__ counts, int Nmax,
-                                                        int* __restrict__ order,
-                                                        float* __restrict__ sboxes,
-                                                        int* __restrict__ sidx) {
-  extern __shared__ __attribute__((aligned(16))) unsigned char dsm[];
-  u64* keys = reinterpret_cast<u64*>(dsm);
-  __shared__ float red[16];
-  const int img = blockIdx.x;
+#define NMS_TILE 16384
+
+__device__ __forceinline__ float prep_max_plus_one(const float* __restrict__ bx, int n, float* red) {
   const int tid = threadIdx.x;
-  int n = counts ? counts[img] : Nmax;
-  if (n > Nmax) n = Nmax;
-  const float* bx = boxes + (size_t)img * Nmax * 4;
-  const float* sc = scores + (size_t)img * Nmax;
-  const int* ix = idxs ? idxs + (size_t)img * Nmax : nullptr;
-
   float m = -INFINITY;
   for (int i = tid; i < n * 4; i += 1024) {
     float v = bx[i];
@@ -48,14 +33,26 @@
     if (tid == 0) red[0] = v;
   }
   __syncthreads();
-  const float maxp1 = red[0] + 1.0f;
-
-  int npad = 1024;
-  while (npad < n) npad <<= 1;
-  if (npad > NPAD) npad = NPAD;
-  for (int i = tid; i < npad; i += 1024)
-    keys[i] = i < n ? (((u64)ordered_desc_key(sc[i]) << 32) | (unsigned)i) : ~0ull;
-  __syncthreads();
+  return red[0] + 1.0f;
+}
+
+__device__ __forceinline__ void prep_gather(const u64* keys, int nrows, const float* __restrict__ bx, const int* __restrict__ ix,
+                                            float maxp1, int* __restrict__ ord, float* __restrict__ sb, int* __restrict__ si) {
+  for (int r = threadIdx.x; r < nrows; r += 1024) {
+    int i = (int)(keys[r] & 0xFFFFFFFFu);
+    ord[r] = i;
+    int id = ix ? ix[i] : 0;
+    float off = (float)id * maxp1;
+    sb[r * 4 + 0] = bx[i * 4 + 0] + off;
+    sb[r * 4 + 1] = bx[i * 4 + 1] + off;
+    sb[r * 4 + 2] = bx[i * 4 + 2] + off;
+    sb[r * 4 + 3] = bx[i * 4 + 3] + off;
+    si[r] = id;
+  }
+}
+
+__device__ __forceinline__ void bitonic_sort_keys(u64* keys, int npad) {
+  const int tid = threadIdx.x;
   for (int k = 2; k <= npad; k <<= 1) {
     for (int j = k >> 1; j > 0; j >>= 1) {
       for (int t = tid; t < npad / 2; t += 1024) {
@@ -68,24 +65,131 @@
       __syncthreads();
     }
   }
+}
+
+__device__ __forceinline__ void prep_sort_all(u64* keys, int n, int npad_max, const float* __restrict__ bx,
+                                              const float* __restrict__ sc, const int* __restrict__ ix, float maxp1,
+                                              int* __restrict__ ord, float* __restrict__ sb, int* __restrict__ si) {
+  const int tid = threadIdx.x;
+  int npad = 1024;
+  while (npad < n) npad <<= 1;
+  if (npad > npad_max) npad = npad_max;
+  for (int i = tid; i < npad; i += 1024)
+    keys[i] = i < n ? (((u64)ordered_desc_key(sc[i]) << 32) | (unsigned)i) : ~0ull;
+  __syncthreads();
+  bitonic_sort_keys(keys, npad);
+  prep_gather(keys, n, bx, ix, maxp1, ord, sb, si);
+}
+
+template <int NPAD>
+__global__ __launch_bounds__(1024) void nms_prep_kernel(const float* __restrict__ boxes,
+                                                        const float* __restrict__ scores,
+                                                        const int* __restrict__ idxs,
+                                                        const int* __restrict__ counts, int Nmax,
+                                                        int* __restrict__ order,
+                                                        float* __restrict__ sboxes,
+                                                        int* __restrict__ sidx, const int* __restrict__ num_keep,
+                                                        int max_keep, int head, const int* __restrict__ full_flag,
+                                                        int* __restrict__ rest_flag) {
+  extern __shared__ __attribute__((aligned(16))) unsigned char dsm[];
+  u64* keys = reinterpret_cast<u64*>(dsm);
+  __shared__ float red[16];
+  const int img = blockIdx.x;
+  int n = counts ? counts[img] : Nmax;
+  if (n > Nmax) n = Nmax;
+  if (num_keep) {
+    const bool run = num_keep[img] < max_keep && n > head && !full_flag[img];
+    if (threadIdx.x == 0) rest_flag[img] = run ? 1 : 0;
+    if (!run) return;
+  }
+  const float* bx = boxes + (size_t)img * Nmax * 4;
+  const float* sc = scores + (size_t)img * Nmax;
+  const int* ix = idxs ? idxs + (size_t)img * Nmax : nullptr;
+  const float maxp1 = prep_max_plus_one(bx, n, red);
+  prep_sort_all(keys, n, NPAD, bx, sc, ix, maxp1, order + (size_t)img * Nmax, sboxes + (size_t)img * Nmax * 4,
+                sidx + (size_t)img * Nmax);
+}
+
+#define NMS_SEL_BITS 12
+#define NMS_SEL_BINS (1 << NMS_SEL_BITS)
+#define NMS_SEL_CAP 4096
+__global__ __launch_bounds__(1024) void nms_head_select_kernel(const float* __restrict__ boxes, const float* __restrict__ scores,
+                                                               const int* __restrict__ idxs, const int* __restrict__ counts,
+                                                               int Nmax, int head, int* __restrict__ order,
+                                                               float* __restrict__ sboxes, int* __restrict__ sidx,
+                                                               int* __restrict__ num_keep, int* __restrict__ full_flag) {
+  extern __shared__ __attribute__((aligned(16))) unsigned char dsm[];
+  u64* keys = reinterpret_cast<u64*>(dsm);
+  __shared__ int hist[NMS_SEL_BINS];
+  __shared__ float red[16];
+  __shared__ int sh[20];
+  __shared__ int s_cnt;
+  const int img = blockIdx.x, tid = threadIdx.x, lane = tid & 63, wave = tid >> 6;
+  int n = counts ? counts[img] : Nmax;
+  if (n > Nmax) n = Nmax;
+  if (n < 0) n = 0;
+  const float* bx = boxes + (size_t)img * Nmax * 4;
+  const float* sc = scores + (size_t)img * Nmax;
+  const int* ix = idxs ? idxs + (size_t)img * Nmax : nullptr;
   int* ord = order + (size_t)img * Nmax;
   float* sb = sboxes + (size_t)img * Nmax * 4;
   int* si = sidx + (size_t)img * Nmax;
-  for (int r = tid; r < n; r += 1024) {
-    int i = (int)(keys[r] & 0xFFFFFFFFu);
-    ord[r] = i;
-    int id = ix ? ix[i] : 0;
-    float off = (float)id * maxp1;
-    sb[r * 4 + 0] = bx[i * 4 + 0] + off;
-    sb[r * 4 + 1] = bx[i * 4 + 1] + off;
-    sb[r * 4 + 2] = bx[i * 4 + 2] + off;
-    sb[r * 4 + 3] = bx[i * 4 + 3] + off;
-    si[r] = id;
-  }
+  if (tid == 0) { num_keep[img] = 0; s_cnt = 0; }
+  if (n == 0) { if (tid == 0) full_flag[img] = 0; return; }
+  for (int i = tid; i < NMS_SEL_BINS; i += 1024) hist[i] = 0;
+  const float maxp1 = prep_max_plus_one(bx, n, red);
+  for (int i = tid; i < n; i += 1024) atomicAdd(&hist[ordered_desc_key(sc[i]) >> (32 - NMS_SEL_BITS)], 1);
+  __syncthreads();
+  const int hk = head < n ? head : n;
+  const int h0 = hist[tid * 4], h1 = hist[tid * 4 + 1], h2 = hist[tid * 4 + 2], h3 = hist[tid * 4 + 3];
+  const int mine = h0 + h1 + h2 + h3;
+  int x = mine;
+#pragma unroll
+  for (int o = 1; o < 64; o <<= 1) {
+    const int t = __shfl_up(x, o);
+    if (lane >= o) x += t;
+  }
+  if (lane == 63) sh[wave] = x;
+  __syncthreads();
+  int ex = x - mine;
+  for (int w = 0; w < wave; ++w) ex += sh[w];
+  if (ex < hk && hk <= ex + mine) {
+    int c = ex, bin = 0;
+    if (c + h0 < hk) { c += h0; bin = 1; if (c + h1 < hk) { c += h1; bin = 2; if (c + h2 < hk) { c += h2; bin = 3; } } }
+    sh[17] = tid * 4 + bin;
+    sh[18] = c + (bin == 0 ? h0 : bin == 1 ? h1 : bin == 2 ? h2 : h3);
+  }
+  __syncthreads();
+  const unsigned int tbin = (unsigned int)sh[17];
+  const int m = sh[18];
+  if (m > NMS_SEL_CAP) {
+    if (tid == 0) full_flag[img] = 1;
+    prep_sort_all(keys, n, NMS_TILE, bx, sc, ix, maxp1, ord, sb, si);
+    return;
+  }
+  if (tid == 0) full_flag[img] = 0;
+  int npad = 1024;
+  while (npad < m) npad <<= 1;
+  for (int i = m + tid; i < npad; i += 1024) keys[i] = ~0ull;
+  for (int i0 = 0; i0 < n; i0 += 1024) {
+    const int i = i0 + tid;
+    const unsigned int key = i < n ? ordered_desc_key(sc[i]) : 0xFFFFFFFFu;
+    const bool hit = i < n && (key >> (32 - NMS_SEL_BITS)) <= tbin;
+    const u64 bal = __ballot(hit);
+    if (bal) {
+      int base = 0;
+      if (lane == 0) base = atomicAdd(&s_cnt, __popcll(bal));
+      base = __shfl(base, 0);
+      const int slot = base + __popcll(bal & ((1ull << lane) - 1ull));
+      if (hit && slot < NMS_SEL_CAP) keys[slot] = ((u64)key << 32) | (unsigned)i;
+    }
+  }
+  __syncthreads();
+  bitonic_sort_keys(keys, npad);
+  prep_gather(keys, hk, bx, ix, maxp1, ord, sb, si);
 }
 
 #define NMS_MASK_STRIDE 96
-#define NMS_TILE 16384
 #define NMS_HEAD_MIN 2048
 __global__ __launch_bounds__(64) void nms_mask_kernel(const float* __restrict__ sboxes,
                                                       const int* __restrict__ sidx,
@@ -460,12 +564,27 @@
   if (Nmax > NMS_TILE)
     per += (long long)Nmax * 4 + NMS_MAX_WORDS * 8 + pad_pow2_ll(Nmax) * 8 + 16;
   else if (Nmax > NMS_HEAD_MIN)
-    per += (long long)Nmax * 4 + NMS_MAX_WORDS * 8 + 16;
+    per += (long long)Nmax * 4 + NMS_MAX_WORDS * 8 + 16 + 8;
   return (long long)B * per + 512;
+}
+
+static long long nms_head_form_offset(int B, int Nmax) {
+  const long long rows_cap = Nmax < NMS_TILE ? Nmax : NMS_TILE, nwords = (rows_cap + 63) / 64;
+  long long o = (long long)B * Nmax * 16 + (long long)B * Nmax * 4 + (long long)B * Nmax * 4;
+  o = (o + 15) & ~15ll;
+  return o + (long long)B * rows_cap * nwords * 8;
+}
+extern "C" long long lvc_batched_nms_flag_offset(int B, int Nmax) {
+  long long o = nms_head_form_offset(B, Nmax) + (long long)B * Nmax * 4;
+  o = (o + 15) & ~15ll;
+  return o + (long long)B * NMS_MAX_WORDS * 8;
 }
 
 static int g_nms_reduce_global = 0;
 extern "C" void lvc_set_nms_reduce_global(int on) { g_nms_reduce_global = on; }
+static int g_selection_fallback = 0;
+extern "C" void lvc_set_selection_fallback(int on) { g_selection_fallback = on; }
+extern "C" int lvc_get_selection_fallback(void) { return g_selection_fallback; }
 
 extern "C" int lvc_batched_nms(const float* boxes, const float* scores, const int* idxs,
                                const int* d_counts, int B, int Nmax, double iou_threshold,
@@ -501,26 +620,40 @@
     (void)hipFuncSetAttribute((const void*)nms_prep_kernel<NP>, hipFuncAttributeMaxDynamicSharedMemorySize, \
                         (int)lds);                                                                   \
     hipLaunchKernelGGL(nms_prep_kernel<NP>, dim3(B), dim3(1024), lds, st, boxes, scores, idxs,       \
-                       d_counts, Nmax, order, sboxes, sidx);                                         \
-  }
-    switch (npad) {
-      case 1024: LAUNCH_PREP(1024); break;
-      case 2048: LAUNCH_PREP(2048); break;
-      case 4096: LAUNCH_PREP(4096); break;
-      case 8192: LAUNCH_PREP(8192); break;
-      default: LAUNCH_PREP(16384); break;
-    }
-#undef LAUNCH_PREP
-    LVC_CHECK_LAUNCH();
+                       d_counts, Nmax, order, sboxes, sidx, gate_nk, max_keep, gate_head, gate_full, gate_rest); \
+  }
+#define LAUNCH_PREP_NPAD()                                                                           \
+    switch (npad) {                                                                                  \
+      case 1024: LAUNCH_PREP(1024); break;                                                           \
+      case 2048: LAUNCH_PREP(2048); break;                                                           \
+      case 4096: LAUNCH_PREP(4096); break;                                                           \
+      case 8192: LAUNCH_PREP(8192); break;                                                           \
+      default: LAUNCH_PREP(16384); break;                                                            \
+    }
+    const int* gate_nk = nullptr; const int* gate_full = nullptr; int* gate_rest = nullptr; int gate_head = 0;
     int head = ((8 * max_keep + 63) / 64) * 64;
     if (head < 1024) head = 1024;
-    if (Nmax > NMS_HEAD_MIN && head * 2 <= Nmax) {
+    const bool head_form = Nmax > NMS_HEAD_MIN && head * 2 <= Nmax;
+    if (!head_form || g_selection_fallback) {
+      LAUNCH_PREP_NPAD();
+      LVC_CHECK_LAUNCH();
+    }
+    if (head_form) {
       int* kept_pos = (int*)ws; ws += (size_t)B * Nmax * 4;
       ws = (char*)(((uintptr_t)ws + 15) & ~(uintptr_t)15);
       u64* removed_init = (u64*)ws;
-      if (hipMemsetAsync(d_num_keep, 0, sizeof(int) * B, st) != hipSuccess) {
-        lvc_set_error("%s: hipMemsetAsync failed", __func__);
-        return LVC_ERR_HIP;
+      int* flags = (int*)((char*)workspace + lvc_batched_nms_flag_offset(B, Nmax));
+      if (g_selection_fallback) {
+        if (hipMemsetAsync(d_num_keep, 0, sizeof(int) * B, st) != hipSuccess) {
+          lvc_set_error("%s: hipMemsetAsync failed", __func__);
+          return LVC_ERR_HIP;
+        }
+      } else {
+        const size_t hlds = lds > (size_t)NMS_SEL_CAP * 8 ? lds : (size_t)NMS_SEL_CAP * 8;
+        (void)hipFuncSetAttribute((const void*)nms_head_select_kernel, hipFuncAttributeMaxDynamicSharedMemorySize, (int)hlds);
+        hipLaunchKernelGGL(nms_head_select_kernel, dim3(B), dim3(1024), hlds, st, boxes, scores, idxs, d_counts, Nmax, head,
+                           order, sboxes, sidx, d_num_keep, flags);
+        LVC_CHECK_LAUNCH();
       }
       const int hw = head / 64;
       hipLaunchKernelGGL(nms_mask_kernel, dim3(hw < NMS_MASK_STRIDE ? hw : NMS_MASK_STRIDE, hw, B), dim3(64), 0, st, sboxes, sidx,
@@ -529,6 +662,11 @@
       hipLaunchKernelGGL(nms_reduce_kernel, dim3(B), dim3(64), 0, st, mask, order, d_counts, Nmax, hw, max_keep, keep,
                          d_num_keep, 0, head, removed_init, kept_pos, 1);
       LVC_CHECK_LAUNCH();
+      if (!g_selection_fallback) {
+        gate_nk = d_num_keep; gate_full = flags; gate_rest = flags + B; gate_head = head;
+        LAUNCH_PREP_NPAD();
+        LVC_CHECK_LAUNCH();
+      }
       const int rest = Nmax - head, rw = (rest + 63) / 64;
       hipLaunchKernelGGL(nms_cross_kernel, dim3(lvc_cdiv(rw, 4), B), dim3(256), 0, st, sboxes, sidx, d_counts, Nmax, rw,
                          iou_threshold, kept_pos, d_num_keep, max_keep, head, rest, removed_init);
@@ -541,6 +679,8 @@
       LVC_CHECK_LAUNCH();
       return LVC_OK;
     }
+#undef LAUNCH_PREP_NPAD
+#undef LAUNCH_PREP
     hipLaunchKernelGGL(nms_mask_kernel, mask_grid, dim3(64), 0, st, sboxes, sidx, d_counts, Nmax, nwords, iou_threshold,
                        mask, 0, rows_cap, (const int*)nullptr, max_keep);
     LVC_CHECK_LAUNCH();
diff --git a/lvc_amd/kernels.py b/lvc_amd/kernels.py
--- a/lvc_amd/kernels.py
+++ b/lvc_amd/kernels.py
@@ -1109,7 +1109,7 @@
     return outs
 
 
-def batched_nms_batch(boxes, scores, idxs, counts, iou_threshold, max_keep=0):
+def batched_nms_batch(boxes, scores, idxs, counts, iou_threshold, max_keep=0, return_flags=False):
     _req_cuda(boxes, scores, idxs, counts)
     B, Nmax = scores.shape
     boxes = boxes.contiguous().float()
@@ -1125,6 +1125,9 @@
         ptr(boxes), ptr(scores), ptr(idxs), ptr(counts), c_int(B), c_int(Nmax), c_double(iou_threshold),
         c_int(max_keep), ptr(keep), ptr(num_keep), ptr(ws), c_longlong(wsb), _stream(boxes))
     check(st, "lvc_batched_nms")
+    if return_flags:
+        off = _lib.lib().lvc_batched_nms_flag_offset(c_int(B), c_int(Nmax))
+        return keep, num_keep, ws[off: off + 8 * B].clone().view(torch.int32).view(2, B)
     return keep, num_keep
 
 
@@ -1149,7 +1152,7 @@
 
 
 def rpn_proposals(logits, deltas, cell_anchors, strides, image_sizes, pre_nms_topk, post_nms_topk,
-                  nms_thresh, min_box_size=0.0):
+                  nms_thresh, min_box_size=0.0, return_flags=False):
     L = len(logits)
     B, A = logits[0].shape[0], cell_anchors[0].shape[0]
     dev = logits[0].device
@@ -1181,6 +1184,9 @@
                                c_float(min_box_size), c_float(SCALE_CLAMP), ptr(boxes), ptr(olog), ptr(count),
                                ptr(ws), c_longlong(nbytes), _stream(boxes))
     check(rc, "lvc_rpn_proposals")
+    if return_flags:
+        off = lib.lvc_rpn_proposals_flag_offset(c_int(B), c_int(L), c_int(A), hs, ws_, c_int(pre_nms_topk))
+        return boxes, olog, count, ws[off: off + 4 * B * L].clone().view(torch.int32).view(B, L)
     return boxes, olog, count
 
 
```

New measurement: 654.1 img/s, median of 6. Within noise of the previous version (+0.6%).
